# jerry102102102/RL_brain_trainer

Measured on AMD Instinct MI355X. Metric: env-steps/sec (whole node), Stage-5 Approach->Finisher PPO loops (rollout + update); value = the Approach loop, finisher.value = the Finisher loop, higher is better.
Workload: dtype f32

## Files before the change

### include/kp1_ppo.h

```cpp
#ifndef KP1_PPO_H
#define KP1_PPO_H

#include <stdint.h>

#include "kp1.h"

#ifdef __cplusplus
extern "C" {
#endif

int kp1_gae_scan(int32_t device, const float* rewards, const float* values, const uint8_t* dones, const float* last_values,
                 float gamma, float gae_lambda, float* advantages, float* returns, int32_t T, int32_t N, void* stream);

int kp1_gae_scan_replicas(int32_t device, const float* rewards, const float* values, const uint8_t* dones, const float* last_values,
                          const float* gamma_lambda, int32_t n_per_replica, float* advantages, float* returns, int32_t T, int32_t N, void* stream);

int kp1_bootstrap_truncated(int32_t device, float* rewards, const float* terminal_values, const uint8_t* dones, float gamma,
                            int64_t count, void* stream);

int kp1_adv_minibatch_sums(int32_t device, const float* advantages, const int64_t* idx, int64_t total, int64_t minibatch, double* out_sums,
                           void* stream);
int kp1_random_permutation(int32_t device, int64_t n, const uint32_t* keys, int64_t* out, void* stream);

int kp1_adv_minibatch_stats(int32_t device, const double* sums, int64_t n_minibatches, float* out_stats, void* stream);

#define KP1_CURRICULUM_MAX_WINDOW 1024
#define KP1_CURRICULUM_MAX_HISTORY 64
typedef struct kp1_curriculum_event {
  int64_t total_timesteps;
  int32_t from_stage, to_stage;
  double trigger_success_rate;
} kp1_curriculum_event;
typedef struct kp1_curriculum_state {
  int32_t stage_index;
  int32_t stage_episode_count;
  int32_t ring_len, ring_head;
  int32_t window_episodes, min_episodes_per_stage, max_stage_index, n_events;
  double success_rate_threshold;
  int64_t num_timesteps;
  int32_t ring[KP1_CURRICULUM_MAX_WINDOW];
  kp1_curriculum_event events[KP1_CURRICULUM_MAX_HISTORY];
} kp1_curriculum_state;

int kp1_curriculum_create(int32_t device, double success_rate_threshold, int32_t window_episodes, int32_t min_episodes_per_stage,
                          int32_t max_stage_index, int32_t initial_stage_index, kp1_curriculum_state** out_dev);
int kp1_curriculum_destroy(int32_t device, kp1_curriculum_state* st_dev);
int kp1_curriculum_observe(int32_t device, kp1_curriculum_state* st_dev, const uint8_t* dones, int32_t n, int32_t steps_per_call, void* stream);
int kp1_curriculum_observe_chunk(int32_t device, kp1_curriculum_state* st_dev, const uint8_t* dones, int32_t n_local, int32_t chunk_steps,
                                 int32_t world, void* stream);
int kp1_curriculum_read(int32_t device, const kp1_curriculum_state* st_dev, kp1_curriculum_state* out_host, void* stream);
int kp1_bind_stage_ptr(kp1_env* env, const int32_t* stage_dev);

#define KP1_CURRICULUM_MAX_REPLICAS 16
int kp1_curriculum_create_population(int32_t device, int32_t n_replicas, double success_rate_threshold, int32_t window_episodes,
                                     int32_t min_episodes_per_stage, int32_t max_stage_index, const int32_t* initial_stages,
                                     kp1_curriculum_state** out_dev);
int kp1_curriculum_observe_population(int32_t device, kp1_curriculum_state* states_dev, const uint8_t* dones, int32_t n_per_replica,
                                      int32_t n_replicas, int32_t steps_per_call, void* stream);
int kp1_curriculum_read_replica(int32_t device, const kp1_curriculum_state* states_dev, int32_t n_replicas, int32_t k,
                                kp1_curriculum_state* out_host, void* stream);
int kp1_bind_population_stages(kp1_env* env, const kp1_curriculum_state* states_dev, int32_t n_replicas);

#define KP1_DOCK_CURRICULUM_MAX_STAGES 16
#define KP1_DOCK_CURRICULUM_MAX_WINDOW 1024
#define KP1_DOCK_CURRICULUM_MAX_HISTORY 32
typedef struct kp1_dock_curriculum_stage {
  double action_delta_scale, dock_residual_action_limit, dock_delta_q_change_limit_scale;
  double close_bucket_probability, close_bucket_min_pos_error_m, close_bucket_max_pos_error_m, close_bucket_max_ori_error_rad,
         handoff_state_probability;
  double close_init_q_noise[KP1_NJ], init_q_noise[KP1_NJ];
  double success_rate_threshold;
  int32_t min_episodes;
  int32_t window_episodes;
  int32_t handoff_offset, handoff_count;
} kp1_dock_curriculum_stage;
typedef struct kp1_dock_curriculum_event {
  int64_t total_timesteps;
  int32_t from_stage, to_stage, stage_episode_count, reserved0;
  double trigger_success_rate;
} kp1_dock_curriculum_event;
typedef struct kp1_dock_curriculum_state {
  int32_t stage_index, stage_episode_count, ring_len, ring_head, window_episodes, n_stages, n_events, reserved0;
  int64_t num_timesteps;
  kp1_dock_curriculum_stage stages[KP1_DOCK_CURRICULUM_MAX_STAGES];
  kp1_dock_curriculum_event events[KP1_DOCK_CURRICULUM_MAX_HISTORY];
  uint8_t ring[KP1_DOCK_CURRICULUM_MAX_WINDOW];
} kp1_dock_curriculum_state;
int kp1_dock_curriculum_create(kp1_env* env, const kp1_dock_curriculum_stage* stages_host, int32_t n_stages, int32_t window_episodes,
                               kp1_dock_curriculum_state** out_dev);
int kp1_dock_curriculum_destroy(kp1_env* env, kp1_dock_curriculum_state* st_dev);
int kp1_dock_curriculum_observe(kp1_env* env, kp1_dock_curriculum_state* st_dev, const uint8_t* dones, int32_t n_local, int32_t chunk_steps, int32_t world,
                                void* stream);
int kp1_dock_curriculum_read(kp1_env* env, const kp1_dock_curriculum_state* st_dev, kp1_dock_curriculum_state* out_host, void* stream);
int kp1_dock_curriculum_create_population(kp1_env* env, const kp1_dock_curriculum_stage* stages_host, int32_t n_stages, int32_t window_episodes,
                                          int32_t n_replicas, kp1_dock_curriculum_state** out_dev);
int kp1_dock_curriculum_observe_population(kp1_env* env, kp1_dock_curriculum_state* states_dev, const uint8_t* dones, int32_t n_per_replica,
                                           int32_t n_replicas, void* stream);
int kp1_dock_curriculum_read_replica(kp1_env* env, const kp1_dock_curriculum_state* states_dev, int32_t n_replicas, int32_t k,
                                     kp1_dock_curriculum_state* out_host, void* stream);

#define KP1_MLP_IN 56
#define KP1_MLP_IN_PAD 64
#define KP1_MLP_IN_ROUTE 80
#define KP1_MLP_IN_ROUTE_PAD 128
#define KP1_MLP_ACT 7

typedef struct kp1_mlp kp1_mlp;

int kp1_mlp_create(int32_t device, int32_t hidden, int32_t max_batch, kp1_mlp** out);
int kp1_mlp_create_ex(int32_t device, int32_t hidden, int32_t obs_dim, int32_t max_batch, kp1_mlp** out);
#define KP1_MLP_MAX_REPLICAS 16
int kp1_mlp_create_population(int32_t device, int32_t hidden, int32_t obs_dim, int32_t max_batch, int32_t replicas, kp1_mlp** out);
int32_t kp1_mlp_replicas(const kp1_mlp* m);
typedef struct kp1_replica_hparams {
  float learning_rate, adam_eps, max_grad_norm, clip_range, ent_coef, vf_coef;
} kp1_replica_hparams;
int kp1_mlp_set_replica_hparams(kp1_mlp* m, const kp1_replica_hparams* host, int32_t n, void* stream);
int kp1_mlp_destroy(kp1_mlp* m);
int64_t kp1_mlp_num_params(int32_t hidden);
int64_t kp1_mlp_num_params_ex(int32_t hidden, int32_t obs_dim);
int kp1_mlp_pack_weights(kp1_mlp* m, const float* params, void* stream);

int kp1_mlp_forward(kp1_mlp* m, const float* obs, int32_t obs_stride, int32_t n, const float* noise, float* mean, float* value,
                    float* action, float* clipped_action, float* log_prob, void* stream);

int kp1_mlp_forward_env_step(kp1_mlp* m, kp1_env* env, const float* obs, int32_t obs_stride, const float* noise, float* value, float* action,
                             float* log_prob, float* next_obs, float* reward, uint8_t* done, float* terminal_obs, void* stream);

int kp1_mlp_loss_grad(kp1_mlp* m, const float* obs, int32_t obs_stride, const int64_t* idx, int32_t n, const float* actions,
                      const float* old_log_prob, const float* advantages, const float* returns, float adv_mean, float adv_inv_std,
                      const float* adv_stats_dev, float clip_range, float ent_coef, float vf_coef, float inv_count, float* grad_out,
                      float* stats_out, int32_t grad_is_zero, void* stream);

#define KP1_MLP_OPT_FUSED 1
#define KP1_MLP_OPT_ACTOR_EXTRA_STEPS 2
#define KP1_MLP_OPT_STEP_COUNT 3
#define KP1_MLP_OPT_PROFILE 4
#define KP1_MLP_OPT_BF16X3_WGRAD 5
#define KP1_MLP_PROFILE_SLOTS 4
#define KP1_MLP_PROFILE_TILE 0
#define KP1_MLP_PROFILE_WGRAD 1
#define KP1_MLP_PROFILE_FINALIZE 2
#define KP1_MLP_PROFILE_ADAM 3
int kp1_mlp_set_option(kp1_mlp* m, int32_t option, int32_t value);
int kp1_mlp_profile_read(kp1_mlp* m, float* out_us , int32_t* out_launches );

int kp1_mlp_adam_step(kp1_mlp* m, float* params, float* grad, float* exp_avg, float* exp_avg_sq, float lr, float eps,
                      float max_grad_norm, int32_t step, int32_t flags, void* stream);

int kp1_mlp_placement_check(int32_t device, int32_t n_rows, int32_t* out, void* stream);
int kp1_mlp_time_kernels(kp1_mlp* m, const float* obs, int32_t obs_stride, int32_t n, int32_t iters, float* out_ms, double* out_flops,
                         void* stream);

int kp1_set_obs_stride(kp1_env* env, int32_t stride);

#ifdef __cplusplus
}
#endif
#endif
```

### rl_brain_trainer_amd/csrc/kp1_env_step.inc

```

#ifdef KP1_ENV_TRACE
constexpr int KP1_ENV_TRACE_SLOTS = 16, KP1_ENV_TRACE_WAVES = 1024;
__device__ unsigned long long kp1_env_trace_buf[KP1_ENV_TRACE_SLOTS * KP1_ENV_TRACE_WAVES];
__device__ __forceinline__ void etr_pin(float v) { asm volatile("" ::"v"(v)); }
__device__ __forceinline__ void etr_pin(double v) { asm volatile("" ::"v"(v)); }
__device__ __forceinline__ void etr_pin(int v) { asm volatile("" ::"v"(v)); }
#define KP1_ETR_PIN(slot, ...)                                                                                                    \
  {                                                                                                                               \
    for (auto pv_ : {__VA_ARGS__}) etr_pin(pv_);                                                                                  \
    __builtin_amdgcn_sched_barrier(0);                                                                                            \
    KP1_ETR(slot)                                                                                                                 \
    __builtin_amdgcn_sched_barrier(0);                                                                                            \
  }
#define KP1_ETR(slot)                                                                                                             \
  {                                                                                                                               \
    const unsigned long long t_ = __builtin_readcyclecounter();                                                                   \
    const int w_ = (int)((blockIdx.x * blockDim.x + threadIdx.x) >> 6);                                                           \
    if ((threadIdx.x & 63) == 0 && w_ < KP1_ENV_TRACE_WAVES) kp1_env_trace_buf[w_ * KP1_ENV_TRACE_SLOTS + (slot)] = t_;           \
  }
#else
#define KP1_ETR(slot)
#define KP1_ETR_PIN(slot, ...)
#endif

// ... 198 lines not shown
    for (int k = 0; k < 6; ++k) goal_pose[k] = (R)opts.goal_pose6[i * 6 + k];
#pragma unroll
    for (int k = 0; k < NJ; ++k) goal_q[k] = (opts.flags & OPT_GOAL_Q) ? (R)opts.goal_q[i * NJ + k] : (R)0;
  } else if (opts.flags & OPT_GOAL_Q) {
#pragma unroll
    for (int k = 0; k < NJ; ++k) {
      gq64[k] = dclip(opts.goal_q[i * NJ + k], smp.lower[k], smp.upper[k]);
      goal_q[k] = (R)gq64[k];
    }
    fk_pose6_kin<R>(cfg.kin.fk, gq64, goal_pose);
  } else if (!given_q) {
#pragma unroll
    for (int k = 0; k < NJ; ++k) goal_q[k] = (R)rs.goal_q[k];
    if (sampled_goal_pose) {
#pragma unroll
      for (int k = 0; k < 6; ++k) goal_pose[k] = (R)rs.goal_pose6[k];
    } else {
      fk_pose6_kin<R>(cfg.kin.fk, rs.goal_q, goal_pose);
    }
  } else {
    rng_load(st.rng64, st.rng32, n, i, rng);
    rng_used = true;
    double g[NJ];
    sample_joint_configuration(smp, rng, smp.goal_sample_margin_fraction, g);
#pragma unroll
    for (int k = 0; k < NJ; ++k) goal_q[k] = (R)g[k];
    fk_pose6_kin<R>(cfg.kin.fk, g, goal_pose);
  }
  if (rng_used) rng_store(st.rng64, st.rng32, n, i, rng);
  R pe[3], oe[3], pn, on;
  pose_error_norms<R>(ee, goal_pose, pe, oe, &pn, &on);
#pragma unroll
  for (int k = 0; k < NJ; ++k) {
    st.q_store(k, i, q64[k]);
    st.r(F_DQ + k, i) = dq[k];
    st.r(F_PREV_ACTION + k, i) = pa[k];
    st.r(F_GOAL_Q + k, i) = goal_q[k];
  }
#pragma unroll
  for (int k = 0; k < 6; ++k) {
    st.r(F_GOAL_POSE + k, i) = goal_pose[k];
    st.r(F_EE_POSE + k, i) = ee[k];
  }
  st.r(F_ENTRY + 0, i) = pn;
  st.r(F_ENTRY + 1, i) = on;
  st.r(F_ENTRY + 2, i) = norm7<R>(pa);
  st.r(F_ENTRY + 3, i) = norm7<R>(dq);
  st.r(F_MIN_POS, i) = std::numeric_limits<R>::infinity();
  st.r(F_POS_ERR, i) = pn;
  st.r(F_ORI_ERR, i) = on;
  st.r(F_EXEC_DQ, i) = (R)0;
  st.r(F_ACTION_L2, i) = (R)0;
  st.r(F_DQ_CHANGE, i) = (R)0;
  st.iv(I_STEP, i) = 0;
  st.iv(I_DWELL, i) = 0;
  st.iv(I_ENTRY, i) = 0;
  st.iv(I_DRIFT, i) = 0;
  st.iv(I_FLAGS, i) = 0;
  st.iv(I_STAGE, i) = have_sample ? rs.stage : stage_index;
  build_observation<R>(cfg, MODE, q, dq, pa, pe, oe, 0, 0, o);
}

template <typename R>
struct StepArgs {
  EnvState<R> st;
  const DevCfg<R>* cfg;
  const DevSampler* smp;
  const kp1_handoff_state* handoff;
  const R* actions;
  float* obs;
  R* reward;
  uint8_t* done;
  float* terminal_obs;
  R* comps;
  int auto_reset;
  int stage_index;
  int obs_stride;
  const int32_t* stage_ptr;
  const kp1_curriculum_state* pop_states;
  int n_per_replica;
  const kp1_dock_curriculum_stage* pop_dock;
};

template <typename R, int MODE, bool COMPS, bool POP = false>
__device__ __forceinline__ void step_env_lane(const StepArgs<R>& a, const int64_t i, const R* __restrict__ act_src, float* __restrict__ o) {
  const int64_t n = a.st.n;
  KP1_ETR(0)
  const DevCfg<R>& __restrict__ cfg = *scalar_cache_warm(a.cfg);
  const DevFk<double>& __restrict__ fkc = cfg.kin.fk;
  KP1_ETR(1)
  const EnvState<R>& st = a.st;
  const R Z = (R)0;

  R act[NJ], dq[NJ], prev_action[NJ], goal[6], ee[6];
  double q[NJ];
#pragma unroll
  for (int k = 0; k < NJ; ++k) {
    act[k] = kp_clip<R>(act_src[k], (R)-1, (R)1);
    q[k] = st.q_loadl(k, i);
    dq[k] = st.rl(F_DQ + k, i);
    prev_action[k] = st.rl(F_PREV_ACTION + k, i);
  }
#pragma unroll
  for (int k = 0; k < 6; ++k) {
    goal[k] = st.rl(F_GOAL_POSE + k, i);
    ee[k] = st.rl(F_EE_POSE + k, i);
  }
  int episode_step = st.ivl(I_STEP, i), dwell = st.ivl(I_DWELL, i), entry_count = st.ivl(I_ENTRY, i), drift_count = st.ivl(I_DRIFT, i);
  int flags = st.ivl(I_FLAGS, i);
  R min_pos = st.rl(F_MIN_POS, i);

  R pe[3], oe[3], prev_pos, prev_ori;
  pose_error_norms<R>(ee, goal, pe, oe, &prev_pos, &prev_ori);
  KP1_ETR_PIN(2, prev_pos, prev_ori)

  constexpr bool LIVE = POP && MODE == KP1_MODE_DOCK;
  const kp1_dock_curriculum_stage* __restrict__ live = nullptr;
  if constexpr (LIVE) live = a.pop_dock + (uint32_t)i / (uint32_t)a.n_per_replica;
  R dyn_limit = kp_clip<R>(cfg.env.dock_residual_action_limit, Z, (R)1);
  R dyn_dqc = kp_max<R>(cfg.env.dock_delta_q_change_limit_scale, Z);
  if constexpr (MODE == KP1_MODE_DOCK) {
    const R residual_limit = LIVE ? (R)live->dock_residual_action_limit : cfg.env.dock_residual_action_limit;
    const R dqc_limit_scale = LIVE ? (R)live->dock_delta_q_change_limit_scale : cfg.env.dock_delta_q_change_limit_scale;
    dyn_limit = kp_clip<R>(interpolate_control<R>(prev_pos, cfg.env.dock_dynamic_action_limit_near_pos_threshold_m,
                                                  cfg.env.dock_dynamic_action_limit_far_pos_threshold_m,
                                                  cfg.env.dock_dynamic_residual_action_limit_near,
                                                  cfg.env.dock_dynamic_residual_action_limit_far, residual_limit), Z, (R)1);
    dyn_dqc = kp_max<R>(interpolate_control<R>(prev_pos, cfg.env.dock_dynamic_action_limit_near_pos_threshold_m,
                                               cfg.env.dock_dynamic_action_limit_far_pos_threshold_m,
                                               cfg.env.dock_dynamic_delta_q_change_limit_scale_near,
                                               cfg.env.dock_dynamic_delta_q_change_limit_scale_far, dqc_limit_scale), Z);
#pragma unroll
    for (int k = 0; k < NJ; ++k) act[k] = kp_clip<R>(act[k], -dyn_limit, dyn_limit);
  }
  const bool prev_in_near = is_near_goal<R>(cfg, prev_pos, prev_ori);
  double scale = LIVE ? live->action_delta_scale : cfg.kin.action_delta_scale;
  if constexpr (MODE == KP1_MODE_DOCK) {
    if (cfg.kin.dock_action_delta_scale > 0.0) scale = cfg.kin.dock_action_delta_scale;
  } else {
    if (cfg.env.dynamic_action_delta_scale_enabled) {
      R mult = interpolate_control<R>(prev_pos, cfg.env.dynamic_action_delta_scale_near_pos_threshold_m,
                                      cfg.env.dynamic_action_delta_scale_far_pos_threshold_m,
                                      cfg.env.dynamic_action_delta_scale_near_multiplier,
                                      cfg.env.dynamic_action_delta_scale_far_multiplier, (R)1);
      scale = cfg.kin.action_delta_scale * (double)kp_max<R>(mult, Z);
    }
  }
  R q_next[NJ], dq_next[NJ];
  double q_next64[NJ];
  R dq_change_ss = Z, dq_ss = Z, prev_dq_ss = Z, act_ss = Z, pact_ss = Z, dact_ss = Z, margin_min = (R)1;
#pragma unroll
  for (int k = 0; k < NJ; ++k) {
    const double max_dq = cfg.kin.dlim[k] * scale;
    double cmd = (double)act[k] * max_dq;
    if constexpr (MODE == KP1_MODE_DOCK) {
      if (dyn_dqc > Z) {
        const double lim = max_dq * (double)dyn_dqc, dqk = (double)dq[k];
        cmd = dqk + dclip(cmd - dqk, -lim, lim);
        cmd = dclip(cmd, -max_dq, max_dq);
      }
    }
    q_next64[k] = joint_clip<double>(q[k] + cmd, cfg.kin.lower[k], cfg.kin.upper[k]);
    q_next[k] = (R)q_next64[k];
    dq_next[k] = (R)(q_next64[k] - q[k]);
    R dd = dq_next[k] - dq[k];
    dq_change_ss += dd * dd;
    dq_ss += dq_next[k] * dq_next[k];
    prev_dq_ss += dq[k] * dq[k];
    act_ss += act[k] * act[k];
    pact_ss += prev_action[k] * prev_action[k];
    R da = act[k] - prev_action[k];
    dact_ss += da * da;
    margin_min = kp_min<R>(margin_min, joint_limit_margin<R>(q_next[k], cfg.lower[k], cfg.upper[k]));
  }
  KP1_ETR_PIN(3, q_next64[0], q_next64[1], q_next64[2], q_next64[3], q_next64[4], q_next64[5], q_next64[6], (double)margin_min, (double)dq_change_ss)
  R ee_next[6];
  fk_pose6_kin<R>(fkc, q_next64, ee_next);
  KP1_ETR_PIN(4, ee_next[0], ee_next[1], ee_next[2], ee_next[3], ee_next[4], ee_next[5])
  R curr_pos, curr_ori;
  pose_error_norms<R>(ee_next, goal, pe, oe, &curr_pos, &curr_ori);
  const bool curr_pre = is_pre_near_goal<R>(cfg, curr_pos, curr_ori);
  const bool curr_near = is_near_goal<R>(cfg, curr_pos, curr_ori);
  min_pos = curr_pos < min_pos ? curr_pos : min_pos;
  if (curr_pre) flags |= FLAG_PRE_NEAR_HIT;
  if (curr_near && !prev_in_near) entry_count += 1;
  dwell = curr_near ? dwell + 1 : 0;
  if (prev_in_near && curr_pos > prev_pos) drift_count += 1;

  const int step_count = episode_step + 1;
  bool terminated = false, truncated = false, success = false, invalid = false;
  const bool criteria = curr_pos <= cfg.term.success_pos_threshold_m &&
                        (!cfg.term.require_orientation || curr_ori <= cfg.term.success_ori_threshold_rad) &&
                        dwell >= cfg.term.success_dwell_steps;
  if (!kp_isfinite(curr_pos) || !kp_isfinite(curr_ori)) {
    terminated = true;
    invalid = true;
  } else if (criteria) {
    success = true;
    if (cfg.term.terminate_on_success) terminated = true;
  }
  if (!terminated && step_count >= cfg.term.max_episode_steps) truncated = true;

  KP1_ETR_PIN(5, curr_pos, curr_ori, (R)dwell, (R)(terminated ? 1 : 0), (R)(truncated ? 1 : 0))
  RewardIn<R> ri;
  ri.prev_pos = prev_pos; ri.curr_pos = curr_pos; ri.prev_ori = prev_ori; ri.curr_ori = curr_ori;
  ri.action_norm = kp_sqrt(act_ss); ri.prev_action_norm = kp_sqrt(pact_ss);
  ri.action_msq = kp_div(act_ss, (R)7); ri.action_delta_msq = kp_div(dact_ss, (R)7);
  ri.dq_norm = kp_sqrt(dq_ss); ri.prev_dq_norm = kp_sqrt(prev_dq_ss); ri.dq_change_l2 = kp_sqrt(dq_change_ss);
  ri.margin_min = margin_min;
  ri.dwell = dwell; ri.entry_count = entry_count; ri.drift_count = drift_count;
  ri.pre = curr_pre; ri.cn = curr_near; ri.pn = prev_in_near; ri.success = success;
  R reward;
  if constexpr (MODE == KP1_MODE_DOCK) {
    ri.entry_pos = st.r(F_ENTRY + 0, i); ri.entry_ori = st.r(F_ENTRY + 1, i);
    ri.entry_action = st.r(F_ENTRY + 2, i); ri.entry_dq = st.r(F_ENTRY + 3, i);
    reward = dock_reward<R, COMPS>(cfg.dock, ri, COMPS ? a.comps + i : nullptr, n);
  } else {
    ri.entry_pos = ri.entry_ori = ri.entry_action = ri.entry_dq = Z;
    reward = approach_reward<R, COMPS>(cfg.reward, ri, COMPS ? a.comps + i : nullptr, n);
  }
  KP1_ETR_PIN(6, reward)
  episode_step += 1;
  if (curr_near) flags |= FLAG_NEAR_HIT;
  flags = success ? (flags | FLAG_SUCCESS) : (flags & ~FLAG_SUCCESS);

  build_observation<R>(cfg, MODE, q_next, dq_next, act, pe, oe, episode_step, dwell, o);
  KP1_ETR_PIN(7, o[0], o[7], o[14], o[21], o[28], o[31], o[34], o[40], o[54], o[55], o[6], o[13], o[20], o[27])
  a.reward[i] = reward;
  const bool done = terminated || truncated;
  a.done[i] = (uint8_t)((terminated ? KP1_DONE_TERMINATED : 0) | (truncated ? KP1_DONE_TRUNCATED : 0) |
                        (success ? KP1_DONE_SUCCESS : 0) | (invalid ? KP1_DONE_INVALID : 0));
  if (done && a.auto_reset) {
    if (a.terminal_obs) store_obs_row(a.terminal_obs, i, o, a.obs_stride);
    ResetOptsDev none = {nullptr, nullptr, nullptr, nullptr, nullptr, 0};
    int stage = a.stage_index;
    const DevSampler& smp = uniform_block(a.smp);
    if constexpr (POP && !LIVE) stage = kp_clipi(a.pop_states[(uint32_t)i / (uint32_t)a.n_per_replica].stage_index, 0, kp_maxi(smp.n_stages - 1, 0));
    else if (a.stage_ptr) stage = kp_clipi(*a.stage_ptr, 0, kp_maxi(smp.n_stages - 1, 0));
    reset_env<R, MODE, LIVE>(st, cfg, smp, a.handoff, none, stage, i, o, live);
    st.r(F_POS_ERR, i) = curr_pos;
    st.r(F_ORI_ERR, i) = curr_ori;
    st.r(F_EXEC_DQ, i) = ri.dq_norm;
    st.r(F_ACTION_L2, i) = ri.action_norm;
    st.r(F_DQ_CHANGE, i) = ri.dq_change_l2;
    st.iv(I_FLAGS, i) = (flags & FLAG_SUCCESS);
  } else {
#pragma unroll
    for (int k = 0; k < NJ; ++k) {
      st.q_store(k, i, q_next64[k]);
      st.r(F_DQ + k, i) = dq_next[k];
      st.r(F_PREV_ACTION + k, i) = act[k];
    }
#pragma unroll
    for (int k = 0; k < 6; ++k) st.r(F_EE_POSE + k, i) = ee_next[k];
    st.r(F_MIN_POS, i) = min_pos;
    st.r(F_POS_ERR, i) = curr_pos;
    st.r(F_ORI_ERR, i) = curr_ori;
    st.r(F_EXEC_DQ, i) = ri.dq_norm;
    st.r(F_ACTION_L2, i) = ri.action_norm;
    st.r(F_DQ_CHANGE, i) = ri.dq_change_l2;
    st.iv(I_STEP, i) = episode_step;
    st.iv(I_DWELL, i) = dwell;
    st.iv(I_ENTRY, i) = entry_count;
    st.iv(I_DRIFT, i) = drift_count;
    st.iv(I_FLAGS, i) = flags;
  }
  KP1_ETR(10)
}
```

### rl_brain_trainer_amd/csrc/kp1_mlp.hip

```cpp
#include <hip/hip_runtime.h>
#include <hip/hip_ext.h>

#include <cmath>
#include <cstddef>
#include <cstdlib>
#include <cstring>
#include <vector>

#include "../../include/kp1_ppo.h"
#include "kp1_device.hpp"
#include "kp1_host.hpp"

using kp1::fail;
using namespace kp1;

typedef float f32x16 __attribute__((ext_vector_type(16)));
typedef float f32x4 __attribute__((ext_vector_type(4)));

namespace {

constexpr int ACT = KP1_MLP_ACT, HEADS = 8;
constexpr float LOG_SQRT_2PI = 0.9189385332046727f;

enum { EPI_BIAS_TANH = 0, EPI_DTANH = 1 };
// ... 974 lines not shown
  __syncthreads();
  for (int k = 128; k > 0; k >>= 1) {
    if (threadIdx.x < k) s[threadIdx.x] += s[threadIdx.x + k];
    __syncthreads();
  }
  if (threadIdx.x == 0) partials[blockIdx.x] = s[0];
}

constexpr int ADAM_BLOCK = 256, VEC = 1;
template <bool POP = false>
__global__ void __launch_bounds__(ADAM_BLOCK) adam_kernel(float* __restrict__ p, float* __restrict__ g, float* __restrict__ m, float* __restrict__ v,
                                                   int64_t n, const double* __restrict__ partials, int n_partials, float lr, float eps, float max_norm,
                                                   float bc1, float bc2_sqrt, const ParamLayout L, const Packed k_, int zero_grad,
                                                   const int* __restrict__ step_counter, int host_step, const int* __restrict__ actor_extra,
                                                   unsigned r_partials, const float* __restrict__ hparams) {
  __shared__ float scale_s;
  const Packed k = POP ? packed_replica(k_, L, blockIdx.y) : k_;
  if constexpr (POP) {
    const unsigned o = blockIdx.y * (unsigned)n;
    p += o; g += o; m += o; v += o;
    partials += blockIdx.y * r_partials;
    if (hparams) {
      const float* e = hparams + blockIdx.y * (unsigned)HP_FIELDS;
      lr = e[HP_LR];
      eps = e[HP_EPS];
      max_norm = e[HP_MAX_NORM];
    }
  }
  const int64_t i0 = ((int64_t)blockIdx.x * ADAM_BLOCK + threadIdx.x) * VEC;
  float g_in[VEC], m_in[VEC], v_in[VEC], p_in[VEC];
#pragma unroll
  for (int j = 0; j < VEC; ++j) {
    const int64_t il = i0 + j < n ? i0 + j : n - 1;
    g_in[j] = g[il]; m_in[j] = m[il]; v_in[j] = v[il]; p_in[j] = p[il];
  }
  const int extra = *actor_extra;
  float base_step = (float)host_step;
  if (step_counter) base_step = (float)*step_counter;
  double s = 0.0;
  if (threadIdx.x < 64) {
    for (int q = threadIdx.x; q < n_partials; q += 64) s += partials[q];
    for (int off = 32; off > 0; off >>= 1) s += __shfl_xor(s, off);
  }
  if (threadIdx.x == 0) {
    const float norm = (float)sqrt(s);
    scale_s = max_norm > 0.f ? fminf(max_norm / (norm + 1e-6f), 1.f) : 1.f;
  }
  if (step_counter) {
    bc1 = 1.f - powf(0.9f, base_step);
    bc2_sqrt = sqrtf(1.f - powf(0.999f, base_step));
  }
  float bc1_a = bc1, bc2_sqrt_a = bc2_sqrt;
  if (extra != 0) {
    const float st = base_step + (float)extra;
    bc1_a = 1.f - powf(0.9f, st);
    bc2_sqrt_a = sqrtf(1.f - powf(0.999f, st));
  }
  __syncthreads();
  const float scale = scale_s;
  float pn[VEC], mn[VEC], vn[VEC];
#pragma unroll
  for (int j = 0; j < VEC; ++j) {
    const int64_t i = i0 + j;
    const bool actor = extra != 0 && ((i >= L.p_w1 && i < L.v_w1) || (i >= L.a_w && i < L.c_w));
    const float b1 = actor ? bc1_a : bc1, b2 = actor ? bc2_sqrt_a : bc2_sqrt;
    const float gi = g_in[j] * scale;
    mn[j] = 0.9f * m_in[j] + 0.1f * gi;
    vn[j] = 0.999f * v_in[j] + 0.001f * gi * gi;
    const float denom = sqrtf(vn[j]) / b2 + eps;
    pn[j] = p_in[j] - (lr / b1) * (mn[j] / denom);
  }
#pragma unroll
  for (int j = 0; j < VEC; ++j) {
    const int64_t i = i0 + j;
    if (i < n) {
      m[i] = mn[j]; v[i] = vn[j]; p[i] = pn[j];
      pack_one(i, pn[j], L, k);
      if (zero_grad) g[i] = 0.f;
    }
  }
}

#include "kp1_env_step.inc"
#include "kp1_mlp_tile.inc"
#include "kp1_mlp_fused.inc"

}

struct kp1_mlp {
  int device = 0, H = 0, Hp = 0, max_batch = 0;
  int K = 1;
  ParamLayout L;
  Packed k{};
  float* h1 = nullptr;
  float* h2 = nullptr;
  float* dz2 = nullptr;
  float* dz1 = nullptr;
  float* xf = nullptr;
  int bf16x3 = 0;
  unsigned short* sp_h1 = nullptr; unsigned short* sp_dz2 = nullptr; unsigned short* sp_dz1 = nullptr; unsigned short* sp_xf = nullptr;
  double* partials = nullptr;
  float* slab = nullptr;
  float* slab1 = nullptr;
  float* bslab = nullptr;
  float* hpart = nullptr;
  int n_finalize_blocks = 0;
  int* step_dev = nullptr;
  float* hparams_dev = nullptr;
  bool hparams_on = false;
  int last_s2_n = 0, last_s1_n = 0;
  int fused = 1;
  const float* last_params = nullptr;
  bool slab_stale = false;
  std::vector<void*> allocs;
  int profile = 0;
  struct ProfPair { hipEvent_t a, b; };
  std::vector<ProfPair> prof[KP1_MLP_PROFILE_SLOTS];
  int prof_used[KP1_MLP_PROFILE_SLOTS] = {0, 0, 0, 0};
};

namespace {
struct ProfSlotInFlight { hipEvent_t a = nullptr, b = nullptr; bool attached = false; };
thread_local ProfSlotInFlight tl_prof;

struct ProfScope {
  kp1_mlp* m; int slot; hipStream_t stream; bool on;
  ProfScope(kp1_mlp* m_, int slot_, hipStream_t s_) : m(m_), slot(slot_), stream(s_), on(m_->profile != 0) {
    if (!on) return;
    auto& v = m->prof[slot];
    if (m->prof_used[slot] >= (int)v.size()) {
      kp1_mlp::ProfPair p{};
      if (hipEventCreate(&p.a) != hipSuccess || hipEventCreate(&p.b) != hipSuccess) { on = false; return; }
      v.push_back(p);
    }
    tl_prof.a = v[m->prof_used[slot]].a;
    tl_prof.b = v[m->prof_used[slot]].b;
    tl_prof.attached = false;
  }
  ~ProfScope() {
    if (!on) return;
    if (!tl_prof.attached) {
      (void)hipEventRecord(tl_prof.a, stream);
      (void)hipEventRecord(tl_prof.b, stream);
    }
    tl_prof = ProfSlotInFlight{};
    m->prof_used[slot] += 1;
  }
};

#define KP1_LAUNCH(kernel, grid, block, bytes, stream, ...)                                                        \
  do {                                                                                                             \
    if (tl_prof.a != nullptr && !tl_prof.attached) {                                                               \
      tl_prof.attached = true;                                                                                     \
      hipExtLaunchKernelGGL(kernel, grid, block, bytes, stream, tl_prof.a, tl_prof.b, 0, __VA_ARGS__);             \
    } else {                                                                                                       \
      hipLaunchKernelGGL(kernel, grid, block, bytes, stream, __VA_ARGS__);                                         \
    }                                                                                                              \
  } while (0)
}

namespace {

constexpr int N_PARTIALS = 128;
constexpr int PARTIALS_STRIDE = 2 * N_PARTIALS + 2048;
constexpr int TN_SPLIT2 = 8, TN_SPLIT1 = 16;

// ... 340 lines not shown
    HIP_TRY(hipMemcpy(m->step_dev + 1, &value, sizeof(int), hipMemcpyHostToDevice));
    return KP1_OK;
  }
  return fail(KP1_ERR_INVALID, "unknown kp1_mlp option");
}

int kp1_mlp_set_replica_hparams(kp1_mlp* m, const kp1_replica_hparams* host, int32_t n, void* stream) {
  static_assert(sizeof(kp1_replica_hparams) == sizeof(float) * HP_FIELDS, "kp1_replica_hparams is HP_FIELDS floats");
  static_assert(offsetof(kp1_replica_hparams, learning_rate) == sizeof(float) * HP_LR && offsetof(kp1_replica_hparams, adam_eps) == sizeof(float) * HP_EPS &&
                offsetof(kp1_replica_hparams, max_grad_norm) == sizeof(float) * HP_MAX_NORM && offsetof(kp1_replica_hparams, clip_range) == sizeof(float) * HP_CLIP &&
                offsetof(kp1_replica_hparams, ent_coef) == sizeof(float) * HP_ENT && offsetof(kp1_replica_hparams, vf_coef) == sizeof(float) * HP_VF,
                "kp1_replica_hparams field order");
  if (!m) return fail(KP1_ERR_INVALID, "NULL argument");
  if (n == 0) {
    m->hparams_on = false;
    return KP1_OK;
  }
  if (m->K == 1) return fail(KP1_ERR_UNSUPPORTED, "a K = 1 handle takes its hyper-parameters as scalar arguments, not a per-replica table");
  if (n != m->K || !host) return fail(KP1_ERR_INVALID, "kp1_mlp_set_replica_hparams needs one entry per replica (n = K)");
  for (int r = 0; r < n; ++r) {
    const kp1_replica_hparams& h = host[r];
    for (float v : {h.learning_rate, h.adam_eps, h.max_grad_norm, h.clip_range, h.ent_coef, h.vf_coef})
      if (!std::isfinite(v)) return fail(KP1_ERR_INVALID, "replica hyper-parameters must be finite");
  }
  int rc = mlp_check_device(m);
  if (rc != KP1_OK) return rc;
  HIP_TRY(hipMemcpyAsync(m->hparams_dev, host, sizeof(kp1_replica_hparams) * (size_t)n, hipMemcpyHostToDevice, (hipStream_t)stream));
  HIP_TRY(hipStreamSynchronize((hipStream_t)stream));
  m->hparams_on = true;
  return KP1_OK;
}

int kp1_mlp_pack_weights(kp1_mlp* m, const float* params, void* stream) {
  if (!m || !params) return fail(KP1_ERR_INVALID, "NULL argument");
  int rc = mlp_check_device(m);
  if (rc != KP1_OK) return rc;
  Packed k = m->k;
  k.formats = PACK_SLAB | PACK_FRAG;
  if (m->K > 1)
    hipLaunchKernelGGL(pack_kernel<true>, dim3((unsigned)((m->L.total + 255) / 256), m->K), dim3(256), 0, (hipStream_t)stream, params, m->L, k);
  else
    hipLaunchKernelGGL(pack_kernel<false>, dim3((unsigned)((m->L.total + 255) / 256)), dim3(256), 0, (hipStream_t)stream, params, m->L, k);
  HIP_TRY(kp1::launch_status());
  m->last_params = params;
  m->slab_stale = false;
  return KP1_OK;
}

int kp1_mlp_forward(kp1_mlp* m, const float* obs, int32_t obs_stride, int32_t n, const float* noise, float* mean, float* value, float* action,
                    float* clipped_action, float* log_prob, void* stream) {
  if (!m || !obs) return fail(KP1_ERR_INVALID, "NULL argument");
  if (n <= 0 || n > m->max_batch) return fail(KP1_ERR_INVALID, "n exceeds the workspace max_batch");
  const int IN = m->L.IN, INP = m->L.INP;
  if (obs_stride != IN && obs_stride != INP) return fail(KP1_ERR_INVALID, "obs_stride must be the observation width or its padded width (56 / 64, or 80 / 128)");
  int rc = mlp_check_device(m);
  if (rc != KP1_OK) return rc;
  if (m->fused && m->Hp == FU_HP) {
    FusedArgs fa{};
    fa.obs = obs; fa.obs_stride = obs_stride; fa.Kreal = obs_stride >= INP ? INP : IN; fa.inp = INP; fa.idx = nullptr; fa.n = n;
    fa.k = m->k;
    fa.noise = noise; fa.mean = mean; fa.value = value; fa.action = action; fa.clipped = clipped_action; fa.log_prob = log_prob;
    rc = launch_fused_infer(fa, (hipStream_t)stream);
    if (rc != KP1_OK) return rc;
    HIP_TRY(kp1::launch_status());
    return KP1_OK;
  }
  rc = launch_forward_layers(m, obs, obs_stride, nullptr, n, (hipStream_t)stream);
  if (rc != KP1_OK) return rc;
  HeadArgs a{};
  a.h2 = m->h2; a.strideH = (int64_t)m->max_batch * m->Hp; a.Hp = m->Hp; a.n = n; a.H = m->H;
  a.w3 = m->k.w3; a.b3 = m->k.b3; a.log_std = m->k.log_std;
  a.noise = noise; a.mean = mean; a.value = value; a.action = action; a.clipped = clipped_action; a.log_prob = log_prob;
  if (m->K > 1) {
    a.r_act = (unsigned)(2 * a.strideH);
    hipLaunchKernelGGL(head_infer_kernel<true>, dim3((n + HEAD_ROWS - 1) / HEAD_ROWS, m->K), dim3(256), sizeof(float) * HEADS * m->Hp, (hipStream_t)stream, a);
  } else {
    hipLaunchKernelGGL(head_infer_kernel<false>, dim3((n + HEAD_ROWS - 1) / HEAD_ROWS), dim3(256), sizeof(float) * HEADS * m->Hp, (hipStream_t)stream, a);
  }
  HIP_TRY(kp1::launch_status());
  return KP1_OK;
}

int kp1_mlp_forward_env_step(kp1_mlp* m, kp1_env* env, const float* obs, int32_t obs_stride, const float* noise, float* value, float* action,
                             float* log_prob, float* next_obs, float* reward, uint8_t* done, float* terminal_obs, void* stream) {
  if (!m || !env || !obs || !action || !next_obs || !reward || !done) return fail(KP1_ERR_INVALID, "NULL argument to kp1_mlp_forward_env_step");
  if (m->K > 1) return fail(KP1_ERR_UNSUPPORTED, "kp1_mlp_forward_env_step is not available on population handles");
  if (!(m->fused && m->Hp == FU_HP) || m->L.INP != 64)
    return fail(KP1_ERR_UNSUPPORTED, "kp1_mlp_forward_env_step needs the 2x256 tile kernels and the 56-float observation (padded to 64)");
  if (obs_stride != m->L.IN && obs_stride != m->L.INP) return fail(KP1_ERR_INVALID, "obs_stride must be 56 or 64");
  int rc = mlp_check_device(m);
  if (rc != KP1_OK) return rc;
  FusedArgs fa{};
  int mode = 0, device = 0;
  int64_t n_envs = 0;
  rc = kp1::env_step_args_f32(env, &fa.env, sizeof fa.env, nullptr, next_obs, reward, done, terminal_obs, 1, &mode, &n_envs, &device);
  if (rc != KP1_OK) return rc;
  if (device != m->device) return fail(KP1_ERR_INVALID, "the env handle and the MLP workspace live on different devices");
  if (n_envs > m->max_batch) return fail(KP1_ERR_INVALID, "more envs than the workspace max_batch");
  fa.obs = obs; fa.obs_stride = obs_stride; fa.Kreal = obs_stride >= m->L.INP ? m->L.INP : m->L.IN; fa.inp = m->L.INP; fa.idx = nullptr; fa.n = (int)n_envs;
  fa.k = m->k;
  fa.noise = noise; fa.value = value; fa.action = action; fa.log_prob = log_prob;
  rc = launch_fused_infer_env(fa, mode, (hipStream_t)stream);
  if (rc != KP1_OK) return rc;
  HIP_TRY(kp1::launch_status());
  return KP1_OK;
}

int kp1_mlp_loss_grad(kp1_mlp* m, const float* obs, int32_t obs_stride, const int64_t* idx, int32_t n, const float* actions,
                      const float* old_log_prob, const float* advantages, const float* returns, float adv_mean, float adv_inv_std,
                      const float* adv_stats_dev, float clip_range, float ent_coef, float vf_coef, float inv_count, float* grad_out,
                      float* stats_out, int32_t grad_is_zero, void* stream_) {
  if (!m || !obs || !actions || !old_log_prob || !advantages || !returns || !grad_out) return fail(KP1_ERR_INVALID, "NULL argument");
  if (n <= 0 || n > m->max_batch) return fail(KP1_ERR_INVALID, "n exceeds the workspace max_batch");
  const int IN = m->L.IN, INP = m->L.INP;
  if (obs_stride != IN && obs_stride != INP) return fail(KP1_ERR_INVALID, "obs_stride must be the observation width or its padded width (56 / 64, or 80 / 128)");
  int rc = mlp_check_device(m);
  if (rc != KP1_OK) return rc;
  hipStream_t stream = (hipStream_t)stream_;
  const int Hp = m->Hp, H = m->H;
  const int64_t act_stride = (int64_t)m->max_batch * Hp;
  const ParamLayout& L = m->L;
  (void)grad_is_zero;
  const bool fused = m->fused && Hp == FU_HP;
  const bool pop = m->K > 1;
  if (pop && !idx) return fail(KP1_ERR_INVALID, "population handles gather their rows through idx [K][n]");
  const int64_t hpart_rep = (int64_t)(m->max_batch / 32) * (10 * Hp + 32);
  int adv_mode = 0;
  if (adv_stats_dev) adv_mode = 2;
  else if (adv_inv_std > 0.f) adv_mode = 3;
  else if (adv_inv_std == 0.f) adv_mode = 1;
  if (adv_mode == 1) {
    if (pop)
      hipLaunchKernelGGL(adv_partials_kernel<true>, dim3(N_PARTIALS, m->K), dim3(256), 0, stream, advantages, idx, n, m->partials, (unsigned)PARTIALS_STRIDE);
    else
      hipLaunchKernelGGL(adv_partials_kernel<false>, dim3(N_PARTIALS), dim3(256), 0, stream, advantages, idx, n, m->partials, 0u);
  }
  const int hpart_stride = 10 * Hp + 32;
  if (fused) {
    FusedArgs fa{};
    fa.obs = obs; fa.obs_stride = obs_stride; fa.Kreal = obs_stride >= INP ? INP : IN; fa.inp = INP; fa.idx = idx; fa.n = n;
    fa.k = m->k;
    fa.actions = actions; fa.old_logp = old_log_prob; fa.adv = advantages; fa.ret = returns;
    fa.adv_partials = m->partials; fa.n_adv_partials = N_PARTIALS; fa.adv_stats = adv_stats_dev; fa.adv_mean = adv_mean; fa.adv_inv_std = adv_inv_std;
    fa.adv_mode = adv_mode;
    fa.clip_range = clip_range; fa.vf_coef = vf_coef; fa.inv_count = inv_count;
    fa.h1 = m->h1; fa.dz2 = m->dz2; fa.dz1 = m->dz1; fa.act_stride = act_stride; fa.xf = m->xf;
    fa.bslab = m->bslab; fa.hpart = m->hpart; fa.hpart_stride = hpart_stride;
    if (m->bf16x3) {
      fa.sp_h1 = m->sp_h1; fa.sp_dz2 = m->sp_dz2; fa.sp_dz1 = m->sp_dz1; fa.sp_xf = m->sp_xf;
      fa.sp_plane = (int64_t)2 * m->max_batch * Hp; fa.sp_plane_x = (int64_t)m->max_batch * INP;
    }
    {
      ProfScope ps(m, KP1_MLP_PROFILE_TILE, stream);
      rc = launch_fused(fa, stream);
    }
    if (rc != KP1_OK) return rc;
  } else {
    rc = launch_forward_layers(m, obs, obs_stride, idx, n, stream);
    if (rc != KP1_OK) return rc;
    HeadArgs a{};
    a.h2 = m->h2; a.strideH = act_stride; a.Hp = Hp; a.n = n; a.H = H;
    a.w3 = m->k.w3; a.b3 = m->k.b3; a.log_std = m->k.log_std;
    a.idx = idx; a.actions = actions; a.old_logp = old_log_prob; a.adv = advantages; a.ret = returns;
    a.adv_partials = m->partials; a.n_adv_partials = N_PARTIALS; a.adv_stats = adv_stats_dev; a.adv_mean = adv_mean; a.adv_inv_std = adv_inv_std;
    a.adv_mode = adv_mode;
    a.clip_range = clip_range; a.ent_coef = ent_coef; a.vf_coef = vf_coef; a.inv_count = inv_count;
    a.dz2 = m->dz2;
    a.hpart = m->hpart; a.hpart_stride = hpart_stride;
    a.r_act = (unsigned)(2 * act_stride); a.r_hpart = (unsigned)hpart_rep; a.r_partials = (unsigned)PARTIALS_STRIDE;
    a.hparams = pop && m->hparams_on ? m->hparams_dev : nullptr;
    {
      const dim3 hgrid((n + HEAD_ROWS - 1) / HEAD_ROWS, m->K);
      const size_t hbytes = sizeof(float) * (HEADS * Hp + HEAD_ROWS * 8 + 84 + 2 * HEAD_ROWS * (Hp + 4));
      if (pop) {
        HIP_TRY(hipFuncSetAttribute((const void*)head_train_kernel<128, true>, hipFuncAttributeMaxDynamicSharedMemorySize, (int)hbytes));
        hipLaunchKernelGGL((head_train_kernel<128, true>), hgrid, dim3(256), hbytes, stream, a);
      } else if (Hp == 256) {
        HIP_TRY(hipFuncSetAttribute((const void*)head_train_kernel<256>, hipFuncAttributeMaxDynamicSharedMemorySize, (int)hbytes));
        hipLaunchKernelGGL(head_train_kernel<256>, hgrid, dim3(256), hbytes, stream, a);
      } else {
        HIP_TRY(hipFuncSetAttribute((const void*)head_train_kernel<128>, hipFuncAttributeMaxDynamicSharedMemorySize, (int)hbytes));
        hipLaunchKernelGGL(head_train_kernel<128>, hgrid, dim3(256), hbytes, stream, a);
      }
    }
// ... 321 lines not shown
```

### rl_brain_trainer_amd/csrc/kp1_mlp_tile.inc

```

struct FusedArgs {
  const float* obs; int64_t obs_stride; int Kreal;
  int inp;
  const int64_t* idx; int n;
  Packed k;
  const float* actions; const float* old_logp; const float* adv; const float* ret;
  const double* adv_partials; int n_adv_partials; const float* adv_stats; float adv_mean, adv_inv_std; int adv_mode;
  float clip_range, vf_coef, inv_count;
  float* h1; float* dz2; float* dz1; int64_t act_stride;
  float* xf;
  float* bslab;
  float* hpart; int hpart_stride;
  const float* noise; float* mean; float* value; float* action; float* clipped; float* log_prob;
  int net_base;
  int stagger_ticks, n_cus;
  StepArgs<float> env;
  unsigned short* sp_h1; unsigned short* sp_dz2; unsigned short* sp_dz1; unsigned short* sp_xf; int64_t sp_plane, sp_plane_x;
};

typedef __bf16 bf16x8 __attribute__((ext_vector_type(8)));
struct Split3 { bf16x8 hi, mid, lo; };
__device__ __forceinline__ Split3 split3(const float* v) {
  Split3 o;
#pragma unroll
  for (int j = 0; j < 8; ++j) {
    const __bf16 h = (__bf16)v[j];
    const float r1 = v[j] - (float)h;
    const __bf16 m = (__bf16)r1;
    const float r2 = r1 - (float)m;
    o.hi[j] = h;
    o.mid[j] = m;
    o.lo[j] = (__bf16)r2;
  }
  return o;
}
__device__ __forceinline__ void store_split3(unsigned short* __restrict__ base, int64_t plane, int64_t fi, int ncb, int cb, int lane, const Split3& s) {
  const int64_t at = ((fi * ncb + cb) * 64 + lane) * 8;
  *reinterpret_cast<bf16x8*>(base + at) = s.hi;
  *reinterpret_cast<bf16x8*>(base + plane + at) = s.mid;
  *reinterpret_cast<bf16x8*>(base + 2 * plane + at) = s.lo;
}

__host__ __device__ inline int64_t frag8_at(int64_t b, int64_t col, int64_t C) {
  return ((b >> 3) * (C >> 5) + (col >> 5)) * 256 + ((col & 31) + 32 * ((b & 7) >> 2)) * 4 + (b & 3);
}

__device__ __forceinline__ f32x4 fu_wload(const char* __restrict__ base, unsigned off) {
  const __amdgpu_buffer_rsrc_t r = __builtin_amdgcn_make_buffer_rsrc(const_cast<char*>(base), 0, 0x7fffffff, 0x00020000);
  return __builtin_bit_cast(f32x4, __builtin_amdgcn_raw_buffer_load_b128(r, (int)off, 0, AUX_SC1));
}
constexpr int FU_HP = 256, FU_BKS = 32, FU_AP = FU_HP + 4;
constexpr int FU_STAGE = FU_HP * FU_BKS;
constexpr int FU_BM = 32, FU_NW = 4, FU_CB = 2, FU_NTH = 64 * FU_NW;
constexpr int FU_SCRATCH = 4 * FU_BM * 8 + FU_BM * 8 + FU_NW * 24 + 64;
constexpr int FU_LDS_FLOATS = 2 * FU_BM * FU_AP + HEADS * FU_HP + FU_SCRATCH;
static_assert(FU_LDS_FLOATS * 4 * 2 <= 160 * 1024, "the two training tiles of one CU must fit its LDS");

template <bool TRAIN, int K1S, int ENV = 0, bool SPLIT = false>
__global__ void __launch_bounds__(FU_NTH, ENV ? 1 : 2) mlp_tile_kernel(const FusedArgs a) {
  static_assert(!(TRAIN && ENV), "the env step rides on the inference tile only");
  static_assert(TRAIN || !SPLIT, "split planes are written by the training tile");
  constexpr int NW = FU_NW, CB = FU_CB, BM = FU_BM, NTH = FU_NTH, CW = 32 * CB;
  constexpr int INP = K1S * FU_BKS, FU_XP = INP + 4, GS_L2 = K1S, GS_BW = K1S + 8, GS_END = K1S + 16;
  constexpr int KG = FU_BKS / 8, NB = CB * KG;
  constexpr int L1_REAL_GROUPS = K1S == 2 ? (KP1_MLP_IN + 7) / 8 : (KP1_MLP_IN_ROUTE + 7) / 8;
  extern __shared__ float lds[];
  float* bufA = lds;
  float* bufB = bufA + BM * FU_AP;
  float* w3s = bufB + BM * FU_AP;
  float* dotred = w3s + HEADS * FU_HP;
  float* dout = dotred + 4 * BM * 8;
  float* wsum = dout + BM * 8;
  float* misc = wsum + NW * 24;

  const int z = (int)blockIdx.z + a.net_base;
  const int m0 = blockIdx.x * BM, slot = blockIdx.x;
  const int tid = threadIdx.x, lane = tid & 63, wave = __builtin_amdgcn_readfirstlane(tid >> 6);
  const unsigned lane_off = (unsigned)lane * 16u;
  const char* __restrict__ W1F = reinterpret_cast<const char*>(a.k.w1f + (int64_t)z * K1S * FU_STAGE + wave * NB * 64 * 4);
  const char* __restrict__ W2F = reinterpret_cast<const char*>(a.k.w2f + (int64_t)z * 8 * FU_STAGE + wave * NB * 64 * 4);
  const char* __restrict__ W2TF = reinterpret_cast<const char*>(a.k.w2tf + (int64_t)z * 8 * FU_STAGE + wave * NB * 64 * 4);

  f32x4 bf[3][NB];
#define FU_BLOAD(gs)                                                                                    \
  if ((gs) < GS_END) {                                                                                  \
    const char* p_ = (gs) < GS_L2 ? W1F + (gs) * (FU_STAGE * 4) : ((gs) < GS_BW ? W2F + ((gs) - GS_L2) * (FU_STAGE * 4) : W2TF + ((gs) - GS_BW) * (FU_STAGE * 4)); \
    _Pragma("unroll") for (int q = 0; q < NB; ++q) bf[(gs) % 3][q] = fu_wload(p_, q * 1024 + lane_off); \
  }
  f32x16 acc[CB];
#define FU_INIT_ACC(bias)                                                                               \
  _Pragma("unroll") for (int c = 0; c < CB; ++c)                                                        \
    _Pragma("unroll") for (int e = 0; e < 16; ++e) acc[c][e] = (bias)[c];
#ifdef KP1_TR_HEADS
#define KP1_TR_G2(slot)
#define KP1_TR_HD(slot) KP1_TR(slot)
#else
#define KP1_TR_G2(slot) KP1_TR(slot)
#define KP1_TR_HD(slot)
#endif
#ifdef KP1_FU_NOMFMA
#define FU_MFMA(acc_, a_, b_) acc_[0] += (a_) * (b_);
#else
#define FU_MFMA(acc_, a_, b_) acc_ = __builtin_amdgcn_mfma_f32_32x32x2f32(a_, b_, acc_, 0, 0, 0);
#endif
#ifdef KP1_FU_NOTANH
#define FU_TANH(x) (x)
#else
#define FU_TANH(x) kp_tanh(x)
#endif
#define FU_GEMM(abuf, ap, KT, GS0)                                                                      \
  {                                                                                                     \
    const float* as = (abuf) + (lane & 31) * (ap) + 4 * (lane >> 5);                                     \
    _Pragma("unroll") for (int s = 0; s < (KT); ++s) {                                                  \
      FU_BLOAD((GS0) + s + 2)                                                                           \
      __builtin_amdgcn_sched_barrier(0);                                                                \
      f32x4 av[KG];                                                                                     \
      _Pragma("unroll") for (int kg = 0; kg < KG; ++kg)                                                 \
        av[kg] = *reinterpret_cast<const f32x4*>(as + s * FU_BKS + kg * 8);                              \
      _Pragma("unroll") for (int kg = 0; kg < KG; ++kg)                                                 \
        if (!((GS0) == 0 && s * KG + kg >= L1_REAL_GROUPS))    \
        _Pragma("unroll") for (int i = 0; i < 4; ++i)                                                   \
          _Pragma("unroll") for (int c = 0; c < CB; ++c)                                                \
            FU_MFMA(acc[c], av[kg][i], bf[((GS0) + s) % 3][c * KG + kg][i])                              \
      __builtin_amdgcn_sched_barrier(0);                                                                \
      if ((GS0) == GS_L2) { KP1_TR_G2(7 + s) }                                                          \
    }                                                                                                   \
  }
#define FU_ROW(e) (((e) & 3) + 8 * ((e) >> 2) + 4 * (lane >> 5))
#define FU_COL(c) (wave * CW + (c) * 32 + (lane & 31))
#ifdef KP1_FU_NOSTORE
#define FU_STORE_ACC(dst)
#else
#define FU_STORE_ACC(dst)                                                                               \
  _Pragma("unroll") for (int c = 0; c < CB; ++c)                                                        \
    _Pragma("unroll") for (int g = 0; g < 4; ++g) {                                                     \
      const f32x4 v_ = {acc[c][4 * g], acc[c][4 * g + 1], acc[c][4 * g + 2], acc[c][4 * g + 3]};        \
      *reinterpret_cast<f32x4*>((dst) + ((int64_t)((m0 >> 3) + g) * (FU_HP / 32) + wave * CB + c) * 256 + lane * 4) = v_; \
    }
#endif
// ... 16 lines not shown
      store_split3((dst) + (zoff), (plane), (int64_t)(m0 >> 4) + f_, (C) / 32, cb_, lane, split3(v8_));  \
    }                                                                                                   \
  }
#ifdef KP1_FU_NOSTORE
#define FU_STORE_FRAG(tile, pitch, dst, C)
#else
#define FU_STORE_FRAG(tile, pitch, dst, C)                                                              \
  _Pragma("unroll") for (int q = wave; q < (BM / 8) * ((C) / 32); q += NW) {                            \
    const int g_ = q / ((C) / 32), cb_ = q % ((C) / 32);                                                \
    const float* t_ = (tile) + (8 * g_ + 4 * (lane >> 5)) * (pitch) + 32 * cb_ + (lane & 31);           \
    f32x4 v_;                                                                                           \
    _Pragma("unroll") for (int i = 0; i < 4; ++i) v_[i] = t_[i * (pitch)];                              \
    *reinterpret_cast<f32x4*>((dst) + ((int64_t)((m0 >> 3) + g_) * ((C) / 32) + cb_) * 256 + lane * 4) = v_; \
  }
#endif

  KP1_TR(0)
  if (TRAIN) { KP1_CLK(0, 0) }
  if (TRAIN && a.stagger_ticks > 0) {
    const int linear = blockIdx.x + gridDim.x * blockIdx.z;
    if (linear >= a.n_cus && linear < 2 * a.n_cus) {
      const unsigned long long t0_ = wall_clock64();
      while (wall_clock64() - t0_ < (unsigned long long)a.stagger_ticks) __builtin_amdgcn_s_sleep(16);
    }
  }
  FU_BLOAD(0)
  FU_BLOAD(1)
  __builtin_amdgcn_sched_barrier(0);
  {
    constexpr int XQ = INP / 4, X_LOADS = BM * XQ / NTH;
    constexpr int W3_LOADS = HEADS * FU_HP / 4 / NTH;
    static_assert(X_LOADS >= 1 && X_LOADS * NTH == BM * XQ && W3_LOADS >= 1 && W3_LOADS * NTH == HEADS * FU_HP / 4, "prologue loads must tile the workgroup");
    int64_t xrow[X_LOADS];
    f32x4 xv[X_LOADS], w3v[W3_LOADS];
#pragma unroll
    for (int j = 0; j < X_LOADS; ++j) {
      const int m = min(m0 + (tid + NTH * j) / XQ, a.n - 1);
      xrow[j] = a.idx ? a.idx[m] : (int64_t)m;
    }
#pragma unroll
    for (int j = 0; j < X_LOADS; ++j) {
      const int k = 4 * ((tid + NTH * j) % XQ);
      xv[j] = *reinterpret_cast<const f32x4*>(a.obs + xrow[j] * a.obs_stride + (k < a.Kreal ? k : 0));
    }
#pragma unroll
    for (int j = 0; j < W3_LOADS; ++j) w3v[j] = *reinterpret_cast<const f32x4*>(a.k.w3 + 4 * (tid + NTH * j));
#pragma unroll
    for (int j = 0; j < X_LOADS; ++j) {
      const int f = tid + NTH * j, row = f / XQ, k = 4 * (f % XQ);
      const float keep = (m0 + row < a.n && k < a.Kreal) ? 1.f : 0.f;
      *reinterpret_cast<f32x4*>(bufB + row * FU_XP + k) = xv[j] * keep;
    }
#pragma unroll
    for (int j = 0; j < W3_LOADS; ++j) *reinterpret_cast<f32x4*>(w3s + 4 * (tid + NTH * j)) = w3v[j];
  }
  if (TRAIN && z == 0 && wave == 0) {
    float mean = 0.f, inv_std = 1.f;
    if (a.adv_mode == 1) {
      double ps = 0.0, pss = 0.0;
      for (int k = lane; k < a.n_adv_partials; k += 64) {
        ps += a.adv_partials[2 * k];
        pss += a.adv_partials[2 * k + 1];
      }
      for (int off = 32; off > 0; off >>= 1) {
        ps += __shfl_xor(ps, off);
        pss += __shfl_xor(pss, off);
      }
      const double mu = ps / a.n;
      const double var = a.n > 1 ? fmax((pss - a.n * mu * mu) / (a.n - 1), 0.0) : 0.0;
      mean = (float)mu;
      inv_std = (float)(1.0 / (sqrt(var) + 1e-8));
    } else if (a.adv_mode == 2) {
      mean = a.adv_stats[0];
      inv_std = a.adv_stats[1];
    } else if (a.adv_mode == 3) {
      mean = a.adv_mean;
      inv_std = a.adv_inv_std;
    }
    if (lane == 0) {
      misc[0] = mean;
      misc[1] = inv_std;
    }
  }
  float bias1[CB], bias2[CB];
#pragma unroll
  for (int c = 0; c < CB; ++c) {
    bias1[c] = a.k.b1[z * FU_HP + FU_COL(c)];
    bias2[c] = a.k.b2[z * FU_HP + FU_COL(c)];
  }
  const int l_row = tid >> 3, l_out = tid & 7;
  const bool l_ok = m0 + l_row < a.n;
  const int64_t l_src = a.idx ? a.idx[min(m0 + l_row, a.n - 1)] : (int64_t)min(m0 + l_row, a.n - 1);
  __syncthreads();
  KP1_TR(1)
  constexpr bool fp32_out = !SPLIT;
  if (TRAIN && z == 0 && fp32_out) { FU_STORE_FRAG(bufB, FU_XP, a.xf, INP) }
  if (TRAIN && z == 0) { FU_STORE_FRAG_SPLIT(bufB, FU_XP, a.sp_xf, a.sp_plane_x, (int64_t)0, INP) }

  FU_INIT_ACC(bias1)
  FU_GEMM(bufB, FU_XP, K1S, 0)
#pragma unroll
  for (int c = 0; c < CB; ++c)
#pragma unroll
    for (int e = 0; e < 16; ++e) {
      acc[c][e] = FU_TANH(acc[c][e]);
      bufA[FU_ROW(e) * FU_AP + FU_COL(c)] = acc[c][e];
    }
  if (TRAIN && fp32_out) { FU_STORE_ACC(a.h1 + z * a.act_stride) }
  if (TRAIN) { FU_STORE_ACC_SPLIT(a.sp_h1, a.sp_plane) }
  __syncthreads();
  KP1_TR(2)
  float l_act = 0.f, l_old = 0.f, l_adv = 0.f, l_ret = 0.f, l_b3 = a.k.b3[l_out], l_ls = a.k.log_std[l_out < ACT ? l_out : 0];
  if (TRAIN) {
    if (z == 0) {
      if (l_out < ACT) l_act = a.actions[l_src * ACT + l_out];
      l_old = a.old_logp[l_src];
      l_adv = a.adv[l_src];
    } else {
      l_ret = a.ret[l_src];
    }
  } else if (z == 0 && a.noise && l_ok && l_out < ACT) {
    l_act = a.noise[l_src * ACT + l_out];
  }

  FU_INIT_ACC(bias2)
  FU_GEMM(bufA, FU_AP, 8, GS_L2)
#pragma unroll
  for (int c = 0; c < CB; ++c)
#pragma unroll
    for (int e = 0; e < 16; ++e) bufB[FU_ROW(e) * FU_AP + FU_COL(c)] = FU_TANH(acc[c][e]);
  __syncthreads();
  KP1_TR(3)

  {
    const int row = lane & 31, kq = wave, part = kq * 2 + (lane >> 5);
    const float* hrow = bufB + row * FU_AP + part * 32;
    f32x4 hv[8];
#pragma unroll
    for (int q = 0; q < 8; ++q) hv[q] = *reinterpret_cast<const f32x4*>(hrow + 4 * q);
    auto dot = [&](int o) {
      const float* w = w3s + o * FU_HP + part * 32;
      float s = 0.f;
#pragma unroll
      for (int q = 0; q < 8; ++q) {
        const f32x4 wv = *reinterpret_cast<const f32x4*>(w + 4 * q);
        s = fmaf(hv[q].x, wv.x, s);
        s = fmaf(hv[q].y, wv.y, s);
        s = fmaf(hv[q].z, wv.z, s);
        s = fmaf(hv[q].w, wv.w, s);
      }
      s += __shfl_xor(s, 32);
      if (lane < 32) dotred[(kq * BM + row) * 8 + o] = s;
    };
    if (z == 0) {
#pragma unroll
      for (int o = 0; o < ACT; ++o) dot(o);
    } else {
      dot(7);
    }
  }
  __syncthreads();
  KP1_TR_HD(7)
  if (!TRAIN) {
    const bool mine = z == 0 ? l_out < ACT : l_out == 7;
    float v = 0.f;
    if (mine) {
#pragma unroll
      for (int p = 0; p < 4; ++p) v += dotred[(p * BM + l_row) * 8 + l_out];
      v += l_b3;
    }
    float lp = 0.f;
    if (z == 0) {
      float act = v;
      if (l_ok && l_out < ACT) {
        if (a.mean) a.mean[l_src * ACT + l_out] = v;
        if (a.noise) {
          act = fmaf(expf(l_ls), l_act, v);
          lp = -0.5f * l_act * l_act - l_ls - LOG_SQRT_2PI;
        }
        if (a.action) a.action[l_src * ACT + l_out] = act;
        if (a.clipped) a.clipped[l_src * ACT + l_out] = fminf(fmaxf(act, -1.f), 1.f);
      }
      lp += __shfl_xor(lp, 1);
      lp += __shfl_xor(lp, 2);
      lp += __shfl_xor(lp, 4);
      if (l_ok && l_out == 0 && a.log_prob) a.log_prob[l_src] = lp;
      if constexpr (ENV != 0) {
        dout[l_row * 8 + l_out] = (l_ok && l_out < ACT) ? act : 0.f;
        __syncthreads();
        if (wave == 0) {
          const bool live = lane < BM && m0 + lane < a.n;
          float o[KP1_OBS_DIM];
          if (live) step_env_lane<float, ENV == 1 ? KP1_MODE_APPROACH : KP1_MODE_DOCK, false>(a.env, (int64_t)(m0 + lane), dout + lane * 8, o);
          store_obs_tile(a.env.obs, (int64_t)m0, min(BM, a.n - m0), o, live, a.env.obs_stride, bufA);
        }
      }
    } else if (l_ok && l_out == 7 && a.value) {
      a.value[l_src] = v;
    }
    return;
  }
  {
    const int row_l = l_row, out = l_out;
    const bool ok = l_ok;
    const bool mine = z == 0 ? out < ACT : out == 7;
    float v = 0.f;
    if (mine) {
#pragma unroll
      for (int p = 0; p < 4; ++p) v += dotred[(p * BM + row_l) * 8 + out];
      v += l_b3;
    }
    float zs = 0.f, inv_sd = 1.f, lp = 0.f;
    if (z == 0 && ok && out < ACT) {
      inv_sd = expf(-l_ls);
      zs = (l_act - v) * inv_sd;
      lp = -0.5f * zs * zs - l_ls - LOG_SQRT_2PI;
    }
    lp += __shfl_xor(lp, 1);
    lp += __shfl_xor(lp, 2);
    lp += __shfl_xor(lp, 4);
    float g_logp = 0.f, d = 0.f, pl = 0.f, vl = 0.f, kl = 0.f;
    if (ok && z == 0) {
      const float A = (l_adv - misc[0]) * misc[1];
      const float lr_ = lp - l_old;
      const float ratio = expf(lr_);
      const float rc = fminf(fmaxf(ratio, 1.f - a.clip_range), 1.f + a.clip_range);
      const float s1 = ratio * A, s2 = rc * A;
      const bool inside = ratio >= 1.f - a.clip_range && ratio <= 1.f + a.clip_range;
      g_logp = (inside || s1 < s2) ? -A * ratio * a.inv_count : 0.f;
      if (out < ACT) {
        d = g_logp * zs * inv_sd;
      } else {
        pl = -fminf(s1, s2);
        kl = (ratio - 1.f) - lr_;
      }
    } else if (ok && out == 7) {
      d = a.vf_coef * 2.f * (v - l_ret) * a.inv_count;
      vl = (l_ret - v) * (l_ret - v);
    }
    dout[row_l * 8 + out] = (ok && mine) ? d : 0.f;
    float gls = (z == 0 && ok && out < ACT) ? g_logp * (zs * zs - 1.f) : 0.f;
    float dsum = (ok && mine) ? d : 0.f;
    float l0 = pl, l1 = vl, l2 = kl;
#pragma unroll
    for (int off = 8; off < 64; off <<= 1) {
      gls += __shfl_xor(gls, off);
      dsum += __shfl_xor(dsum, off);
      l0 += __shfl_xor(l0, off);
      l1 += __shfl_xor(l1, off);
      l2 += __shfl_xor(l2, off);
    }
    if (lane < 8) {
      wsum[wave * 24 + out] = dsum;
      wsum[wave * 24 + 8 + out] = gls;
      if (out == 7) {
        wsum[wave * 24 + 16] = l0;
        wsum[wave * 24 + 17] = l1;
        wsum[wave * 24 + 18] = l2;
      }
    }
  }
  KP1_TR_HD(8)
  __syncthreads();
  KP1_TR_HD(9)
  if (tid < 18) {
    const int k = tid;
    const int w = k < 8 ? k : (k < 15 ? 8 + (k - 8) : 16 + (k - 15));
    const float v = ((wsum[w] + wsum[24 + w]) + wsum[48 + w]) + wsum[72 + w];
    const bool pi_slot = (k < 7) || (k >= 8 && k < 15) || k == 15 || k == 17;
    if (pi_slot == (z == 0)) a.hpart[(int64_t)slot * a.hpart_stride + 10 * FU_HP + k] = v;
  }
  {
    constexpr int DZ_COLS = FU_HP / NW, DZ_CG = DZ_COLS / 4, DZ_RG = 64 / DZ_CG, DZ_ROWS = 32 / DZ_RG;
    const int cg = lane % DZ_CG, rg = lane / DZ_CG, col = wave * DZ_COLS + 4 * cg;
    float* part = a.hpart + (int64_t)slot * a.hpart_stride;
    f32x4 gw[ACT], gb2 = {0.f, 0.f, 0.f, 0.f}, w3c[ACT];
#pragma unroll
// ... 102 lines not shown
```

### rl_brain_trainer_amd/csrc/kp1_ppo.hip

```cpp
#include <hip/hip_runtime.h>

#include <cstring>
#include <vector>

#include "../../include/kp1_ppo.h"
#include "kp1_host.hpp"

using kp1::fail;

namespace {

__global__ void __launch_bounds__(256) gae_scan_kernel(const float* __restrict__ rewards, const float* __restrict__ values,
                                                       const uint8_t* __restrict__ dones, const float* __restrict__ last_values,
                                                       float gamma, float lam, float* __restrict__ adv, float* __restrict__ ret, int T, int N) {
  const int i = blockIdx.x * blockDim.x + threadIdx.x;
  if (i >= N) return;
  float next_value = last_values[i];
  float last_gae = 0.0f;
  for (int t = T - 1; t >= 0; --t) {
    const int64_t k = (int64_t)t * N + i;
    const float nonterm = (dones[k] & (KP1_DONE_TERMINATED | KP1_DONE_TRUNCATED)) ? 0.0f : 1.0f;
    const float v = values[k];
    const float delta = rewards[k] + gamma * next_value * nonterm - v;
    last_gae = delta + gamma * lam * nonterm * last_gae;
    adv[k] = last_gae;
    ret[k] = last_gae + v;
    next_value = v;
  }
}

__global__ void __launch_bounds__(256) gae_scan_replicas_kernel(const float* __restrict__ rewards, const float* __restrict__ values,
                                                                const uint8_t* __restrict__ dones, const float* __restrict__ last_values,
                                                                const float* __restrict__ gamma_lambda, int n_per_replica, float* __restrict__ adv,
                                                                float* __restrict__ ret, int T, int N) {
  const int i = blockIdx.x * blockDim.x + threadIdx.x;
  if (i >= N) return;
  const int r = i / n_per_replica;
  const float gamma = gamma_lambda[2 * r], lam = gamma_lambda[2 * r + 1];
  float next_value = last_values[i];
  float last_gae = 0.0f;
  for (int t = T - 1; t >= 0; --t) {
    const int64_t k = (int64_t)t * N + i;
    const float nonterm = (dones[k] & (KP1_DONE_TERMINATED | KP1_DONE_TRUNCATED)) ? 0.0f : 1.0f;
    const float v = values[k];
    const float delta = rewards[k] + gamma * next_value * nonterm - v;
    last_gae = delta + gamma * lam * nonterm * last_gae;
    adv[k] = last_gae;
    ret[k] = last_gae + v;
    next_value = v;
  }
}

__global__ void __launch_bounds__(256) bootstrap_kernel(float* __restrict__ rewards, const float* __restrict__ tv,
                                                        const uint8_t* __restrict__ dones, float gamma, int64_t count) {
  const int64_t k = (int64_t)blockIdx.x * blockDim.x + threadIdx.x;
  if (k >= count) return;
  const uint8_t d = dones[k];
  if ((d & KP1_DONE_TRUNCATED) && !(d & KP1_DONE_TERMINATED)) rewards[k] += gamma * tv[k];
}

struct TrackerCtx {
  int stage, count, len, head, window, min_episodes, max_stage, n_events, sum;
  double threshold;
  long long timesteps;
  bool ring_dirty;
};

__device__ __forceinline__ void tracker_load(const kp1_curriculum_state* __restrict__ st, int* __restrict__ ring, TrackerCtx& c) {
  const int lane = threadIdx.x;
  c.stage = st->stage_index; c.count = st->stage_episode_count; c.len = st->ring_len; c.head = st->ring_head;
  c.window = st->window_episodes; c.min_episodes = st->min_episodes_per_stage; c.max_stage = st->max_stage_index; c.n_events = st->n_events;
  c.threshold = st->success_rate_threshold; c.timesteps = st->num_timesteps;
  c.ring_dirty = false;
  int part = 0;
  for (int k = lane; k < c.window; k += 64) {
    const int v = st->ring[k];
    ring[k] = v;
    const int age = k >= c.head ? k - c.head : k - c.head + c.window;
    if (age < c.len) part += v;
  }
  for (int off = 32; off > 0; off >>= 1) part += __shfl_xor(part, off);
  c.sum = part;
  __syncthreads();
}

__device__ __forceinline__ void tracker_store(kp1_curriculum_state* __restrict__ st, const int* __restrict__ ring, const TrackerCtx& c) {
  const int lane = threadIdx.x;
  __syncthreads();
  if (c.ring_dirty)
    for (int k = lane; k < c.window; k += 64) st->ring[k] = ring[k];
  if (lane == 0) {
    st->stage_index = c.stage; st->stage_episode_count = c.count; st->ring_len = c.len; st->ring_head = c.head;
    st->n_events = c.n_events; st->num_timesteps = c.timesteps;
  }
}

constexpr int TRK_BLOCK = 64 * 64, TRK_PARALLEL_MIN = 192;
struct TrackerScratch { uint8_t* sbit; uint16_t* pfx; };

__device__ __forceinline__ void tracker_append_run(int* __restrict__ ring, TrackerCtx& c, const uint8_t* __restrict__ sbit, int pos, int R) {
  const int lane = threadIdx.x, W = c.window;
  const int j0 = R > W ? R - W : 0;
  __syncthreads();
  for (int j = j0 + lane; j < R; j += 64) ring[(c.head + c.len + j) % W] = sbit[pos + j];
  __syncthreads();
  const int over = c.len + R - W;
  c.head = over > 0 ? (c.head + over) % W : c.head;
  c.len = c.len + R < W ? c.len + R : W;
  c.count += R;
  int part = 0;
  for (int k = lane; k < W; k += 64) {
    const int age = k >= c.head ? k - c.head : k - c.head + W;
    if (age < c.len) part += ring[k];
  }
  for (int off = 32; off > 0; off >>= 1) part += __shfl_xor(part, off);
  c.sum = part;
}

__device__ __forceinline__ void tracker_block_parallel(kp1_curriculum_state* __restrict__ st, int* __restrict__ ring, TrackerCtx& c, const TrackerScratch& ws,
                                                       unsigned long long dmask, unsigned long long smask, int E) {
  const int lane = threadIdx.x, W = c.window;
  int mine = __popcll(dmask), off = mine;
  for (int d = 1; d < 64; d <<= 1) {
    const int up = __shfl_up(off, d);
    if (lane >= d) off += up;
  }
  off -= mine;
  __syncthreads();
  for (unsigned long long m = dmask; m; m &= m - 1) {
    const int b = __ffsll((long long)m) - 1;
    ws.sbit[off++] = (uint8_t)((smask >> b) & 1ull);
  }
  __syncthreads();
  int pos = 0;
  while (pos < E) {
    const int R = E - pos;
    if (c.stage >= c.max_stage) {
      tracker_append_run(ring, c, ws.sbit, pos, R);
      break;
    }
    const int L = c.len, T = L + R;
    const int seg = (T + 63) / 64, j_lo = lane * seg < T ? lane * seg : T, j_hi = j_lo + seg < T ? j_lo + seg : T;
    auto y = [&](int j) -> int { return j < L ? ring[(c.head + j) % W] : (int)ws.sbit[pos + (j - L)]; };
    int tot = 0;
    for (int j = j_lo; j < j_hi; ++j) tot += y(j);
    int run = tot;
    for (int d = 1; d < 64; d <<= 1) {
      const int up = __shfl_up(run, d);
      if (lane >= d) run += up;
    }
    run -= tot;
    __syncthreads();
    if (lane == 0) ws.pfx[0] = 0;
    for (int j = j_lo; j < j_hi; ++j) {
      run += y(j);
      ws.pfx[j + 1] = (uint16_t)run;
    }
    __syncthreads();
    int best = R;
    for (int r = lane; r < R; r += 64) {
      const int filled = L + r + 1;
      if (filled < W || c.count + r + 1 < c.min_episodes) continue;
      const int wsum = (int)ws.pfx[filled] - (int)ws.pfx[filled - W];
      if ((double)wsum / (double)W >= c.threshold) {
        best = r;
        break;
      }
    }
    for (int d = 32; d > 0; d >>= 1) {
      const int o = __shfl_xor(best, d);
      best = o < best ? o : best;
    }
    if (best >= R) {
      tracker_append_run(ring, c, ws.sbit, pos, R);
      break;
    }
    const int filled = L + best + 1;
    const double rate = (double)((int)ws.pfx[filled] - (int)ws.pfx[filled - W]) / (double)W;
    if (lane == 0 && c.n_events < KP1_CURRICULUM_MAX_HISTORY) {
      kp1_curriculum_event& ev = st->events[c.n_events];
      ev.total_timesteps = c.timesteps;
      ev.from_stage = c.stage;
      ev.to_stage = c.stage + 1;
      ev.trigger_success_rate = rate;
    }
    c.n_events += 1;
    c.stage += 1;
    c.count = 0;
    c.len = 0;
    c.head = 0;
    c.sum = 0;
    pos += best + 1;
  }
}

__device__ __forceinline__ void curriculum_scan(kp1_curriculum_state* __restrict__ st, int* __restrict__ ring, TrackerCtx& c, const TrackerScratch& ws,
                                                const uint8_t* __restrict__ dones, int n, int steps_per_call) {
  const int lane = threadIdx.x;
  c.timesteps += steps_per_call;
  for (int base = 0; base < n; base += 64 * 64) {
    const int first = base + lane * 64;
    unsigned long long dmask = 0ull, smask = 0ull;
    if (first + 64 <= n && (reinterpret_cast<uintptr_t>(dones + first) & 15) == 0) {
      const uint4* p = reinterpret_cast<const uint4*>(dones + first);
      uint4 w[4];
#pragma unroll
      for (int q = 0; q < 4; ++q) w[q] = p[q];
#pragma unroll
      for (int q = 0; q < 4; ++q) {
        const unsigned int words[4] = {w[q].x, w[q].y, w[q].z, w[q].w};
#pragma unroll
        for (int k = 0; k < 4; ++k)
#pragma unroll
          for (int b = 0; b < 4; ++b) {
            const unsigned int d = (words[k] >> (8 * b)) & 0xffu;
            const int bit = q * 16 + k * 4 + b;
            if (d & (KP1_DONE_TERMINATED | KP1_DONE_TRUNCATED)) {
              dmask |= 1ull << bit;
              if (d & KP1_DONE_SUCCESS) smask |= 1ull << bit;
            }
          }
      }
    } else {
      for (int b = 0; b < 64 && first + b < n; ++b) {
        const uint8_t d = dones[first + b];
        if (d & (KP1_DONE_TERMINATED | KP1_DONE_TRUNCATED)) {
          dmask |= 1ull << b;
          if (d & KP1_DONE_SUCCESS) smask |= 1ull << b;
        }
      }
    }
    unsigned long long busy = __ballot(dmask != 0ull);
    if (busy == 0ull) continue;
    c.ring_dirty = true;
    {
      int ended = __popcll(dmask);
      for (int off = 32; off > 0; off >>= 1) ended += __shfl_xor(ended, off);
      if (ended >= TRK_PARALLEL_MIN) {
        tracker_block_parallel(st, ring, c, ws, dmask, smask, ended);
        continue;
      }
    }
    int stage = c.stage, count = c.count, len = c.len, head = c.head, sum = c.sum, n_events = c.n_events;
    const int window = c.window;
    while (busy) {
      const int src = __ffsll((long long)busy) - 1;
      busy &= busy - 1;
      unsigned long long m = __shfl(dmask, src);
      const unsigned long long sm = __shfl(smask, src);
      if (lane != 0) continue;
      while (m) {
        const int b = __ffsll((long long)m) - 1;
        m &= m - 1;
        const int success = (int)((sm >> b) & 1ull);
        count += 1;
        if (len < window) {
          ring[head + len < window ? head + len : head + len - window] = success;
          len += 1;
          sum += success;
        } else {
          sum += success - ring[head];
          ring[head] = success;
          head = head + 1 < window ? head + 1 : 0;
        }
        if (stage >= c.max_stage) continue;
        if (count < c.min_episodes) continue;
        if (len < window) continue;
        const double rate = (double)sum / (double)len;
        if (rate >= c.threshold) {
          if (n_events < KP1_CURRICULUM_MAX_HISTORY) {
            kp1_curriculum_event& ev = st->events[n_events];
            ev.total_timesteps = c.timesteps;
            ev.from_stage = stage;
            ev.to_stage = stage + 1;
            ev.trigger_success_rate = rate;
          }
          n_events += 1;
          stage += 1;
          count = 0;
          len = 0;
          head = 0;
          sum = 0;
        }
      }
    }
    c.stage = __shfl(stage, 0); c.count = __shfl(count, 0); c.len = __shfl(len, 0); c.head = __shfl(head, 0);
    c.sum = __shfl(sum, 0); c.n_events = __shfl(n_events, 0);
  }
}

__global__ void __launch_bounds__(64) curriculum_kernel(kp1_curriculum_state* __restrict__ st, const uint8_t* __restrict__ dones, int n,
                                                        int steps_per_call) {
  __shared__ int ring[KP1_CURRICULUM_MAX_WINDOW];
  __shared__ uint8_t sbit[TRK_BLOCK];
  __shared__ uint16_t pfx[TRK_BLOCK + KP1_CURRICULUM_MAX_WINDOW + 1];
  const TrackerScratch ws = {sbit, pfx};
  {
    const int lane = threadIdx.x;
    bool any = false;
    for (int base = 0; base < n; base += 64 * 64) {
      const int first = base + lane * 64;
      if (first + 64 <= n && (reinterpret_cast<uintptr_t>(dones + first) & 15) == 0) {
        const uint4* p = reinterpret_cast<const uint4*>(dones + first);
        unsigned int acc = 0u;
#pragma unroll
        for (int q = 0; q < 4; ++q) {
          const uint4 w = p[q];
          acc |= w.x | w.y | w.z | w.w;
        }
        any |= (acc & (0x01010101u * (unsigned)(KP1_DONE_TERMINATED | KP1_DONE_TRUNCATED))) != 0u;
      } else {
        for (int b = 0; b < 64 && first + b < n; ++b) any |= (dones[first + b] & (KP1_DONE_TERMINATED | KP1_DONE_TRUNCATED)) != 0;
      }
    }
    if (__ballot(any) == 0ull) {
      if (lane == 0) atomicAdd(reinterpret_cast<unsigned long long*>(&st->num_timesteps), (unsigned long long)(long long)steps_per_call);
      return;
    }
  }
  TrackerCtx c;
  tracker_load(st, ring, c);
  curriculum_scan(st, ring, c, ws, dones, n, steps_per_call);
  tracker_store(st, ring, c);
}

__global__ void __launch_bounds__(64) curriculum_chunk_kernel(kp1_curriculum_state* __restrict__ st, const uint8_t* __restrict__ dones, int n_local,
                                                              int chunk_steps, int world, int steps_per_env_step) {
  __shared__ int ring[KP1_CURRICULUM_MAX_WINDOW];
  __shared__ uint8_t sbit[TRK_BLOCK];
  __shared__ uint16_t pfx[TRK_BLOCK + KP1_CURRICULUM_MAX_WINDOW + 1];
  const TrackerScratch ws = {sbit, pfx};
  TrackerCtx c;
  tracker_load(st, ring, c);
  for (int t = 0; t < chunk_steps; ++t)
    for (int r = 0; r < world; ++r)
      curriculum_scan(st, ring, c, ws, dones + ((int64_t)r * chunk_steps + t) * n_local, n_local, r == 0 ? steps_per_env_step : 0);
  tracker_store(st, ring, c);
}

__global__ void __launch_bounds__(64) curriculum_population_kernel(kp1_curriculum_state* __restrict__ states, const uint8_t* __restrict__ dones_all,
                                                                   int n, int steps_per_call) {
  __shared__ int ring[KP1_CURRICULUM_MAX_WINDOW];
  __shared__ uint8_t sbit[TRK_BLOCK];
  __shared__ uint16_t pfx[TRK_BLOCK + KP1_CURRICULUM_MAX_WINDOW + 1];
  const TrackerScratch ws = {sbit, pfx};
  kp1_curriculum_state* __restrict__ st = states + blockIdx.x;
  const uint8_t* __restrict__ dones = dones_all + (int64_t)blockIdx.x * n;
  {
    const int lane = threadIdx.x;
    bool any = false;
    for (int base = 0; base < n; base += 64 * 64) {
      const int first = base + lane * 64;
      if (first + 64 <= n && (reinterpret_cast<uintptr_t>(dones + first) & 15) == 0) {
        const uint4* p = reinterpret_cast<const uint4*>(dones + first);
        unsigned int acc = 0u;
#pragma unroll
        for (int q = 0; q < 4; ++q) {
          const uint4 w = p[q];
          acc |= w.x | w.y | w.z | w.w;
        }
        any |= (acc & (0x01010101u * (unsigned)(KP1_DONE_TERMINATED | KP1_DONE_TRUNCATED))) != 0u;
      } else {
        for (int b = 0; b < 64 && first + b < n; ++b) any |= (dones[first + b] & (KP1_DONE_TERMINATED | KP1_DONE_TRUNCATED)) != 0;
      }
    }
    if (__ballot(any) == 0ull) {
      if (lane == 0) atomicAdd(reinterpret_cast<unsigned long long*>(&st->num_timesteps), (unsigned long long)(long long)steps_per_call);
      return;
    }
  }
  TrackerCtx c;
  tracker_load(st, ring, c);
  curriculum_scan(st, ring, c, ws, dones, n, steps_per_call);
  tracker_store(st, ring, c);
}

int check_device(int device) {
  int count = 0;
  if (hipGetDeviceCount(&count) != hipSuccess || count <= 0) return fail(KP1_ERR_NO_DEVICE, "no HIP device: this library has no CPU path");
  if (device < 0 || device >= count) return fail(KP1_ERR_INVALID, "device index out of range");
  HIP_TRY(hipSetDevice(device));
  return KP1_OK;
}

}

extern "C" {

int kp1_gae_scan(int32_t device, const float* rewards, const float* values, const uint8_t* dones, const float* last_values, float gamma,
                 float gae_lambda, float* advantages, float* returns, int32_t T, int32_t N, void* stream) {
  if (!rewards || !values || !dones || !last_values || !advantages || !returns || T <= 0 || N <= 0) return fail(KP1_ERR_INVALID, "bad argument to kp1_gae_scan");
  int rc = check_device(device);
  if (rc != KP1_OK) return rc;
  const int block = N <= 16384 ? 64 : 256;
  hipLaunchKernelGGL(gae_scan_kernel, dim3((N + block - 1) / block), dim3(block), 0, (hipStream_t)stream, rewards, values, dones, last_values,
                     gamma, gae_lambda, advantages, returns, T, N);
  HIP_TRY(kp1::launch_status());
  return KP1_OK;
}

int kp1_gae_scan_replicas(int32_t device, const float* rewards, const float* values, const uint8_t* dones, const float* last_values,
                          const float* gamma_lambda, int32_t n_per_replica, float* advantages, float* returns, int32_t T, int32_t N, void* stream) {
  if (!rewards || !values || !dones || !last_values || !gamma_lambda || !advantages || !returns || T <= 0 || N <= 0)
    return fail(KP1_ERR_INVALID, "bad argument to kp1_gae_scan_replicas");
  if (n_per_replica <= 0 || N % n_per_replica != 0) return fail(KP1_ERR_INVALID, "kp1_gae_scan_replicas: N must be a multiple of n_per_replica");
  int rc = check_device(device);
  if (rc != KP1_OK) return rc;
  const int block = N <= 16384 ? 64 : 256;
  hipLaunchKernelGGL(gae_scan_replicas_kernel, dim3((N + block - 1) / block), dim3(block), 0, (hipStream_t)stream, rewards, values, dones,
                     last_values, gamma_lambda, n_per_replica, advantages, returns, T, N);
  HIP_TRY(kp1::launch_status());
  return KP1_OK;
}

}

namespace {
__global__ void __launch_bounds__(256) adv_minibatch_sums_kernel(const float* __restrict__ adv, const int64_t* __restrict__ idx, int64_t total, int64_t mb,
                                                                 double* __restrict__ out) {
  __shared__ double s1[256], s2[256];
  const int64_t begin = (int64_t)blockIdx.x * mb, end = begin + mb < total ? begin + mb : total;
  double a = 0.0, b = 0.0;
  for (int64_t i = begin + threadIdx.x; i < end; i += 256) {
    const double v = (double)adv[idx ? idx[i] : i];
    a += v;
    b += v * v;
  }
  s1[threadIdx.x] = a;
  s2[threadIdx.x] = b;
  __syncthreads();
  for (int k = 128; k > 0; k >>= 1) {
    if (threadIdx.x < k) {
      s1[threadIdx.x] += s1[threadIdx.x + k];
      s2[threadIdx.x] += s2[threadIdx.x + k];
    }
    __syncthreads();
  }
  if (threadIdx.x == 0) {
    out[3 * blockIdx.x] = s1[0];
    out[3 * blockIdx.x + 1] = s2[0];
    out[3 * blockIdx.x + 2] = (double)(end - begin);
  }
}
struct PermKeys { uint32_t mul[4], add[4]; };
__global__ void __launch_bounds__(256) permutation_kernel(int64_t* __restrict__ out, int64_t n, int bits, const PermKeys k) {
  const int64_t i = (int64_t)blockIdx.x * 256 + threadIdx.x;
  if (i >= n) return;
  const uint32_t mask = bits >= 32 ? 0xffffffffu : ((1u << bits) - 1u);
  const int sh = bits > 1 ? bits / 2 : 1;
  uint32_t x = (uint32_t)i;
  do {
#pragma unroll
    for (int r = 0; r < 4; ++r) {
      x = (x * k.mul[r] + k.add[r]) & mask;
      x ^= x >> sh;
    }
  } while ((int64_t)x >= n);
// ... 24 lines not shown
  while (((int64_t)1 << bits) < n) ++bits;
  PermKeys k;
  for (int r = 0; r < 4; ++r) {
    k.mul[r] = keys[r] | 1u;
    k.add[r] = keys[4 + r];
  }
  hipLaunchKernelGGL(permutation_kernel, dim3((unsigned)((n + 255) / 256)), dim3(256), 0, (hipStream_t)stream, out, n, bits, k);
  HIP_TRY(kp1::launch_status());
  return KP1_OK;
}

int kp1_adv_minibatch_stats(int32_t device, const double* sums, int64_t n_minibatches, float* out_stats, void* stream) {
  if (!sums || !out_stats || n_minibatches <= 0) return fail(KP1_ERR_INVALID, "bad argument to kp1_adv_minibatch_stats");
  int rc = check_device(device);
  if (rc != KP1_OK) return rc;
  hipLaunchKernelGGL(adv_minibatch_stats_kernel, dim3((unsigned)((n_minibatches + 63) / 64)), dim3(64), 0, (hipStream_t)stream, sums, n_minibatches,
                     out_stats);
  HIP_TRY(kp1::launch_status());
  return KP1_OK;
}

int kp1_adv_minibatch_sums(int32_t device, const float* advantages, const int64_t* idx, int64_t total, int64_t minibatch, double* out_sums,
                           void* stream) {
  if (!advantages || !out_sums || total <= 0 || minibatch <= 0) return fail(KP1_ERR_INVALID, "bad argument to kp1_adv_minibatch_sums");
  int rc = check_device(device);
  if (rc != KP1_OK) return rc;
  const int64_t n_mb = (total + minibatch - 1) / minibatch;
  hipLaunchKernelGGL(adv_minibatch_sums_kernel, dim3((unsigned)n_mb), dim3(256), 0, (hipStream_t)stream, advantages, idx, total, minibatch, out_sums);
  HIP_TRY(kp1::launch_status());
  return KP1_OK;
}

int kp1_bootstrap_truncated(int32_t device, float* rewards, const float* terminal_values, const uint8_t* dones, float gamma, int64_t count,
                            void* stream) {
  if (!rewards || !terminal_values || !dones || count <= 0) return fail(KP1_ERR_INVALID, "bad argument to kp1_bootstrap_truncated");
  int rc = check_device(device);
  if (rc != KP1_OK) return rc;
  hipLaunchKernelGGL(bootstrap_kernel, dim3((unsigned)((count + 255) / 256)), dim3(256), 0, (hipStream_t)stream, rewards, terminal_values, dones,
                     gamma, count);
  HIP_TRY(kp1::launch_status());
  return KP1_OK;
}

int kp1_curriculum_create(int32_t device, double success_rate_threshold, int32_t window_episodes, int32_t min_episodes_per_stage,
                          int32_t max_stage_index, int32_t initial_stage_index, kp1_curriculum_state** out_dev) {
  return kp1_curriculum_create_population(device, 1, success_rate_threshold, window_episodes, min_episodes_per_stage, max_stage_index,
                                          &initial_stage_index, out_dev);
}
int kp1_curriculum_create_population(int32_t device, int32_t n_replicas, double success_rate_threshold, int32_t window_episodes,
                                     int32_t min_episodes_per_stage, int32_t max_stage_index, const int32_t* initial_stages,
                                     kp1_curriculum_state** out_dev) {
  if (!out_dev || !initial_stages) return fail(KP1_ERR_INVALID, "NULL argument");
  if (n_replicas < 1 || n_replicas > KP1_CURRICULUM_MAX_REPLICAS) return fail(KP1_ERR_INVALID, "n_replicas must be in [1, KP1_CURRICULUM_MAX_REPLICAS]");
  int rc = check_device(device);
  if (rc != KP1_OK) return rc;
  std::vector<kp1_curriculum_state> h((size_t)n_replicas);
  for (int k = 0; k < n_replicas; ++k) {
    kp1_curriculum_state& s = h[(size_t)k];
    std::memset(&s, 0, sizeof s);
    s.success_rate_threshold = success_rate_threshold;
    s.window_episodes = window_episodes < 1 ? 1 : window_episodes;
    if (s.window_episodes > KP1_CURRICULUM_MAX_WINDOW) return fail(KP1_ERR_INVALID, "window_episodes exceeds KP1_CURRICULUM_MAX_WINDOW");
    s.min_episodes_per_stage = min_episodes_per_stage < 1 ? 1 : min_episodes_per_stage;
    s.max_stage_index = max_stage_index < 0 ? 0 : max_stage_index;
    int init = initial_stages[k] < s.max_stage_index ? initial_stages[k] : s.max_stage_index;
    s.stage_index = init < 0 ? 0 : init;
  }
  kp1_curriculum_state* d = nullptr;
  HIP_TRY(hipMalloc((void**)&d, sizeof(kp1_curriculum_state) * h.size()));
  HIP_TRY(hipMemcpy(d, h.data(), sizeof(kp1_curriculum_state) * h.size(), hipMemcpyHostToDevice));
  *out_dev = d;
  return KP1_OK;
}
int kp1_curriculum_destroy(int32_t device, kp1_curriculum_state* st_dev) {
  int rc = check_device(device);
  if (rc != KP1_OK) return rc;
  HIP_TRY(hipFree(st_dev));
  return KP1_OK;
}
int kp1_curriculum_observe(int32_t device, kp1_curriculum_state* st_dev, const uint8_t* dones, int32_t n, int32_t steps_per_call, void* stream) {
  if (!st_dev || !dones || n <= 0) return fail(KP1_ERR_INVALID, "bad argument to kp1_curriculum_observe");
  int rc = check_device(device);
  if (rc != KP1_OK) return rc;
  hipLaunchKernelGGL(curriculum_kernel, dim3(1), dim3(64), 0, (hipStream_t)stream, st_dev, dones, n, steps_per_call);
  HIP_TRY(kp1::launch_status());
  return KP1_OK;
}
int kp1_curriculum_observe_chunk(int32_t device, kp1_curriculum_state* st_dev, const uint8_t* dones, int32_t n_local, int32_t chunk_steps,
                                 int32_t world, void* stream) {
  if (!st_dev || !dones || n_local <= 0 || chunk_steps <= 0 || world <= 0) return fail(KP1_ERR_INVALID, "bad argument to kp1_curriculum_observe_chunk");
  int rc = check_device(device);
  if (rc != KP1_OK) return rc;
  hipLaunchKernelGGL(curriculum_chunk_kernel, dim3(1), dim3(64), 0, (hipStream_t)stream, st_dev, dones, n_local, chunk_steps, world, n_local * world);
  HIP_TRY(kp1::launch_status());
  return KP1_OK;
}
int kp1_curriculum_observe_population(int32_t device, kp1_curriculum_state* states_dev, const uint8_t* dones, int32_t n_per_replica,
                                      int32_t n_replicas, int32_t steps_per_call, void* stream) {
  if (!states_dev || !dones || n_per_replica <= 0 || n_replicas < 1 || n_replicas > KP1_CURRICULUM_MAX_REPLICAS)
    return fail(KP1_ERR_INVALID, "bad argument to kp1_curriculum_observe_population");
  int rc = check_device(device);
  if (rc != KP1_OK) return rc;
  hipLaunchKernelGGL(curriculum_population_kernel, dim3((unsigned)n_replicas), dim3(64), 0, (hipStream_t)stream, states_dev, dones, n_per_replica,
                     steps_per_call);
  HIP_TRY(kp1::launch_status());
  return KP1_OK;
}
int kp1_curriculum_read_replica(int32_t device, const kp1_curriculum_state* states_dev, int32_t n_replicas, int32_t k, kp1_curriculum_state* out_host,
                                void* stream) {
  if (!states_dev || !out_host) return fail(KP1_ERR_INVALID, "NULL argument");
  if (k < 0 || k >= n_replicas) return fail(KP1_ERR_INVALID, "replica index out of range");
  return kp1_curriculum_read(device, states_dev + k, out_host, stream);
}
int kp1_curriculum_read(int32_t device, const kp1_curriculum_state* st_dev, kp1_curriculum_state* out_host, void* stream) {
  if (!st_dev || !out_host) return fail(KP1_ERR_INVALID, "NULL argument");
  int rc = check_device(device);
  if (rc != KP1_OK) return rc;
  HIP_TRY(hipMemcpyAsync(out_host, st_dev, sizeof *out_host, hipMemcpyDeviceToHost, (hipStream_t)stream));
  HIP_TRY(hipStreamSynchronize((hipStream_t)stream));
  return KP1_OK;
}

}
```

### rl_brain_trainer_amd/curriculum.py

```python
from __future__ import annotations

import ctypes as C
from typing import Any, Sequence

import torch

from . import native

MAX_WINDOW = 1024
MAX_HISTORY = 64


class _Event(C.Structure):
    _fields_ = [("total_timesteps", C.c_int64), ("from_stage", C.c_int32), ("to_stage", C.c_int32), ("trigger_success_rate", C.c_double)]


class CurriculumState(C.Structure):
    _fields_ = [
        ("stage_index", C.c_int32), ("stage_episode_count", C.c_int32), ("ring_len", C.c_int32), ("ring_head", C.c_int32),
        ("window_episodes", C.c_int32), ("min_episodes_per_stage", C.c_int32), ("max_stage_index", C.c_int32), ("n_events", C.c_int32),
        ("success_rate_threshold", C.c_double), ("num_timesteps", C.c_int64),
        ("ring", C.c_int32 * MAX_WINDOW), ("events", _Event * MAX_HISTORY),
    ]


class PointCurriculum:
    def __init__(self, *, success_rate_threshold: float, window_episodes: int, min_episodes_per_stage: int, max_stage_index: int,
                 initial_stage_index: int = 0, device: torch.device | int = 0) -> None:
        self.L = native.load()
        self.device = torch.device("cuda", device) if isinstance(device, int) else torch.device(device)
        self._st = C.c_void_p()
        native.check(self.L.kp1_curriculum_create(self.device.index or 0, float(success_rate_threshold), int(window_episodes),
                                                  int(min_episodes_per_stage), int(max_stage_index), int(initial_stage_index), C.byref(self._st)))

    @property
    def stage_ptr(self) -> int:
        return int(self._st.value)

    def attach(self, env) -> None:
        native.check(self.L.kp1_bind_stage_ptr(env._handle, C.c_void_p(self.stage_ptr)))

    def observe(self, dones: torch.Tensor, steps_per_call: int) -> None:
        stream = torch.cuda.current_stream(self.device).cuda_stream
        native.check(self.L.kp1_curriculum_observe(self.device.index or 0, self._st, C.c_void_p(dones.data_ptr()), int(dones.numel()),
                                                   int(steps_per_call), C.c_void_p(stream)))

    def observe_chunk(self, dones_all: torch.Tensor, n_local: int, chunk_steps: int, world: int) -> None:
        assert dones_all.numel() == world * chunk_steps * n_local and dones_all.dtype == torch.uint8 and dones_all.is_contiguous()
        stream = torch.cuda.current_stream(self.device).cuda_stream
        native.check(self.L.kp1_curriculum_observe_chunk(self.device.index or 0, self._st, C.c_void_p(dones_all.data_ptr()), int(n_local), int(chunk_steps),
                                                         int(world), C.c_void_p(stream)))

    def read(self) -> CurriculumState:
        out = CurriculumState()
        stream = torch.cuda.current_stream(self.device).cuda_stream
        native.check(self.L.kp1_curriculum_read(self.device.index or 0, self._st, C.byref(out), C.c_void_p(stream)))
        return out

    def summary(self) -> dict[str, object]:
        return self._summary_of(self.read())

    @staticmethod
    def _summary_of(st: CurriculumState) -> dict[str, object]:
        n = st.ring_len
        recent = [st.ring[k] for k in range(n)]
        return {
            "stage_index": int(st.stage_index),
            "stage_episode_count": int(st.stage_episode_count),
            "recent_success_rate": float(sum(recent)) / float(n) if n else 0.0,
            "history": [
                {"from_stage_index": int(e.from_stage), "to_stage_index": int(e.to_stage),
                 "trigger_success_rate": float(e.trigger_success_rate), "total_timesteps": int(e.total_timesteps)}
                for e in list(st.events)[: min(st.n_events, MAX_HISTORY)]
            ],
        }

    def close(self) -> None:
        if self._st.value:
            self.L.kp1_curriculum_destroy(self.device.index or 0, self._st)
            self._st = C.c_void_p()


class PointCurriculumPopulation(PointCurriculum):

    def __init__(self, *, success_rate_threshold: float, window_episodes: int, min_episodes_per_stage: int, max_stage_index: int,
                 initial_stage_indices: Sequence[int], device: torch.device | int = 0) -> None:
        from .vec_env import MAX_REPLICAS

        stages = [int(s) for s in initial_stage_indices]
        if not 1 <= len(stages) <= MAX_REPLICAS:
            raise ValueError(f"PointCurriculumPopulation holds 1 to {MAX_REPLICAS} trackers (got {len(stages)} initial stages)")
        self.K = len(stages)
        self.env: Any = None
        self.L = native.load()
        self.device = torch.device("cuda", device) if isinstance(device, int) else torch.device(device)
        self._st = C.c_void_p()
        init = (C.c_int32 * self.K)(*stages)
        native.check(self.L.kp1_curriculum_create_population(self.device.index or 0, self.K, float(success_rate_threshold), int(window_episodes),
                                                             int(min_episodes_per_stage), int(max_stage_index), C.cast(init, C.c_void_p),
                                                             C.byref(self._st)))

    @property
    def stage_ptr(self) -> int:
        raise TypeError("a population tracker has one stage per replica: attach() binds all of them to a population env")

    def attach(self, env: Any) -> None:
        if not getattr(env, "is_population", False):
            raise TypeError("PointCurriculumPopulation tracks the replicas of an ArmKinematicPopulationVecEnv")
        if env.n_envs % self.K != 0 or getattr(env, "K", self.K) != self.K:
            raise ValueError(f"a population env of {env.n_envs} envs does not split into this tracker's {self.K} replicas")
        native.check(self.L.kp1_bind_population_stages(env._handle, C.c_void_p(self._st.value), self.K))
        env.launch_args_version += 1
        self.env = env

    def observe(self, dones: torch.Tensor, steps_per_call: int) -> None:
        if dones.numel() % self.K != 0 or dones.dtype != torch.uint8 or not dones.is_contiguous():
            raise ValueError(f"observe() takes the contiguous uint8 done bytes of all {self.K} replicas")
        stream = torch.cuda.current_stream(self.device).cuda_stream
        native.check(self.L.kp1_curriculum_observe_population(self.device.index or 0, self._st, C.c_void_p(dones.data_ptr()), dones.numel() // self.K,
                                                              self.K, int(steps_per_call), C.c_void_p(stream)))

    def observe_chunk(self, dones_all: torch.Tensor, n_local: int, chunk_steps: int, world: int) -> None:
        raise TypeError("the population tracker has no data-parallel form")

    def read(self, k: int = 0) -> CurriculumState:
        out = CurriculumState()
        stream = torch.cuda.current_stream(self.device).cuda_stream
        native.check(self.L.kp1_curriculum_read_replica(self.device.index or 0, self._st, self.K, int(k), C.byref(out), C.c_void_p(stream)))
# ... 28 lines not shown
```

### rl_brain_trainer_amd/mlp.py

```python
from __future__ import annotations

import ctypes as C

import torch

from . import native

OBS_DIM, OBS_PAD, ACT_DIM = 56, 64, 7


def _p(t: torch.Tensor | None):
    return C.c_void_p(t.data_ptr()) if t is not None else None


class MlpKernels:
    def __init__(self, hidden: int, device: torch.device, max_batch: int = 8192, obs_dim: int = OBS_DIM, replicas: int = 1) -> None:
        self.L = native.load()
        L = self.L
        vp, i32, f32 = C.c_void_p, C.c_int32, C.c_float
        L.kp1_mlp_create_ex.argtypes = [i32, i32, i32, i32, C.POINTER(vp)]
        L.kp1_mlp_create_population.argtypes = [i32, i32, i32, i32, i32, C.POINTER(vp)]
        L.kp1_mlp_replicas.argtypes = [vp]
        L.kp1_mlp_replicas.restype = i32
        L.kp1_mlp_destroy.argtypes = [vp]
        L.kp1_mlp_num_params_ex.argtypes = [i32, i32]
        L.kp1_mlp_num_params_ex.restype = C.c_int64
        L.kp1_mlp_pack_weights.argtypes = [vp, vp, vp]
        L.kp1_mlp_forward.argtypes = [vp, vp, i32, i32, vp, vp, vp, vp, vp, vp, vp]
        L.kp1_mlp_forward_env_step.argtypes = [vp, vp, vp, i32, vp, vp, vp, vp, vp, vp, vp, vp, vp]
        L.kp1_mlp_loss_grad.argtypes = [vp, vp, i32, vp, i32, vp, vp, vp, vp, f32, f32, vp, f32, f32, f32, f32, vp, vp, i32, vp]
        L.kp1_mlp_adam_step.argtypes = [vp, vp, vp, vp, vp, f32, f32, f32, i32, i32, vp]
        L.kp1_mlp_time_kernels.argtypes = [vp, vp, i32, i32, i32, vp, vp, vp]
        L.kp1_mlp_placement_check.argtypes = [i32, i32, vp, vp]
        L.kp1_mlp_set_option.argtypes = [vp, i32, i32]
        L.kp1_mlp_profile_read.argtypes = [vp, vp, vp]
        L.kp1_mlp_set_replica_hparams.argtypes = [vp, vp, i32, vp]
        self.hidden = hidden
        self.device = device
        self.max_batch = int(max_batch)
        self._h = vp()
        self.obs_dim = int(obs_dim)
        self.obs_pad = 64 if self.obs_dim <= 64 else 128
        if replicas == 1:
            native.check(L.kp1_mlp_create_ex(device.index or 0, hidden, self.obs_dim, self.max_batch, C.byref(self._h)))
        else:
            native.check(L.kp1_mlp_create_population(device.index or 0, hidden, self.obs_dim, self.max_batch, int(replicas), C.byref(self._h)))
        self.replicas = int(L.kp1_mlp_replicas(self._h))
        self.num_params = int(L.kp1_mlp_num_params_ex(hidden, self.obs_dim))

    def close(self) -> None:
        if self._h.value:
            self.L.kp1_mlp_destroy(self._h)
            self._h = C.c_void_p()

    OPT_FUSED = 1

    def set_fused(self, on: bool) -> None:
        native.check(self.L.kp1_mlp_set_option(self._h, self.OPT_FUSED, int(bool(on))))

    OPT_ACTOR_EXTRA_STEPS = 2

    def set_actor_extra_steps(self, steps: int) -> None:
        native.check(self.L.kp1_mlp_set_option(self._h, self.OPT_ACTOR_EXTRA_STEPS, int(steps)))

    OPT_STEP_COUNT = 3

    def set_step_count(self, steps: int) -> None:
        native.check(self.L.kp1_mlp_set_option(self._h, self.OPT_STEP_COUNT, int(steps)))

    OPT_BF16X3_WGRAD = 5

    def set_bf16x3_wgrad(self, on: bool) -> None:
        native.check(self.L.kp1_mlp_set_option(self._h, self.OPT_BF16X3_WGRAD, int(bool(on))))

    OPT_PROFILE = 4
    PROFILE_SLOTS = ("mlp_train_tile", "gemm_tn_split", "grad_finalize", "adam")

    def set_profile(self, on: bool) -> None:
        native.check(self.L.kp1_mlp_set_option(self._h, self.OPT_PROFILE, int(bool(on))))

    def profile_read(self) -> dict[str, dict[str, float]]:
        us = (C.c_float * 4)()
        cnt = (C.c_int32 * 4)()
        native.check(self.L.kp1_mlp_profile_read(self._h, C.cast(us, C.c_void_p), C.cast(cnt, C.c_void_p)))
        return {name: {"us": float(us[i]), "launches": int(cnt[i])} for i, name in enumerate(self.PROFILE_SLOTS)}

    HPARAM_FIELDS = ("learning_rate", "adam_eps", "max_grad_norm", "clip_range", "ent_coef", "vf_coef")

    def set_replica_hparams(self, rows: list[dict[str, float]] | None) -> None:
        if rows is None:
            native.check(self.L.kp1_mlp_set_replica_hparams(self._h, None, 0, self._stream()))
            return
        table = (C.c_float * (len(rows) * len(self.HPARAM_FIELDS)))(*[float(r[f]) for r in rows for f in self.HPARAM_FIELDS])
        native.check(self.L.kp1_mlp_set_replica_hparams(self._h, C.cast(table, C.c_void_p), len(rows), self._stream()))

    def _stream(self):
        return C.c_void_p(torch.cuda.current_stream(self.device).cuda_stream)

    def pack(self, flat_params: torch.Tensor) -> None:
        assert flat_params.numel() == self.replicas * self.num_params and flat_params.dtype == torch.float32 and flat_params.is_contiguous()
        native.check(self.L.kp1_mlp_pack_weights(self._h, _p(flat_params), self._stream()))

    def forward(self, obs: torch.Tensor, *, noise=None, mean=None, value=None, action=None, clipped=None, log_prob=None) -> None:
        assert obs.shape[0] % self.replicas == 0
        n, stride = obs.shape[0] // self.replicas, obs.shape[1]
        assert obs.is_contiguous() and obs.dtype == torch.float32
        native.check(self.L.kp1_mlp_forward(self._h, _p(obs), stride, n, _p(noise), _p(mean), _p(value), _p(action), _p(clipped), _p(log_prob), self._stream()))

    def forward_env_step(self, env, obs: torch.Tensor, *, noise, value, action, log_prob, next_obs, reward, done, terminal_obs) -> None:
        assert obs.is_contiguous() and obs.dtype == torch.float32 and obs.shape[0] == env.n_envs
        native.check(self.L.kp1_mlp_forward_env_step(self._h, env._handle, _p(obs), obs.shape[1], _p(noise), _p(value), _p(action), _p(log_prob),
                                                     _p(next_obs), _p(reward), _p(done), _p(terminal_obs), self._stream()))

    def mean_value(self, obs: torch.Tensor) -> tuple[torch.Tensor, torch.Tensor]:
        n = obs.shape[0]
        mean = torch.empty((n, ACT_DIM), dtype=torch.float32, device=obs.device)
        value = torch.empty(n, dtype=torch.float32, device=obs.device)
        for s in range(0, n, self.max_batch):
            e = min(s + self.max_batch, n)
            self.forward(obs[s:e], mean=mean[s:e], value=value[s:e])
        return mean, value

    def loss_grad(self, obs: torch.Tensor, idx: torch.Tensor | None, n: int, actions, old_logp, adv, ret, *, clip_range: float, ent_coef: float,
                  vf_coef: float, inv_count: float, grad_out: torch.Tensor, stats_out: torch.Tensor | None, adv_stats: torch.Tensor | None = None,
                  normalize: bool = True, grad_is_zero: bool = False) -> None:
        assert obs.is_contiguous() and grad_out.numel() == self.replicas * self.num_params
        assert self.replicas == 1 or (idx is not None and idx.numel() == self.replicas * n)
        inv_std = 0.0 if normalize else -1.0
        native.check(self.L.kp1_mlp_loss_grad(self._h, _p(obs), obs.shape[-1], _p(idx), n, _p(actions), _p(old_logp), _p(adv), _p(ret), 0.0, inv_std,
                                              _p(adv_stats), clip_range, ent_coef, vf_coef, inv_count, _p(grad_out), _p(stats_out), int(grad_is_zero), self._stream()))

    def adam_step(self, params, grad, exp_avg, exp_avg_sq, *, lr: float, eps: float, max_grad_norm: float, step: int,
                  fused_norm: bool = False) -> None:
        native.check(self.L.kp1_mlp_adam_step(self._h, _p(params), _p(grad), _p(exp_avg), _p(exp_avg_sq), lr, eps, max_grad_norm, step,
                                              2 if fused_norm else 0, self._stream()))

    def placement_check(self, n_rows: int) -> dict[str, int | float]:
        out = (C.c_int32 * 8)()
        native.check(self.L.kp1_mlp_placement_check(self.device.index or 0, int(n_rows), C.cast(out, C.c_void_p), self._stream()))
        wgs, pairs, same, rr, cus, used, arrived, xcds = (int(v) for v in out)
        return {"workgroups": wgs, "compute_units": cus, "compute_units_used": used, "second_tile_on_same_cu": same, "second_tile_pairs": pairs,
                "on_xcd_of_block_index_mod_8": rr, "xcds_among_first_8_blocks": xcds, "all_resident": arrived == wgs}

    def time_kernels(self, obs: torch.Tensor, n: int, iters: int = 20) -> dict[str, dict[str, float]]:
        ms = (C.c_float * 6)()
        fl = (C.c_double * 6)()
        native.check(self.L.kp1_mlp_time_kernels(self._h, _p(obs), obs.shape[-1], n, iters, C.cast(ms, C.c_void_p), C.cast(fl, C.c_void_p), self._stream()))
        names = ("gemm_nt_fwd_l2", "gemm_nt_bwd_dz1", "gemm_tn_dw2", "gemm_nt_fwd_l1", "mlp_train_tile", "gemm_tn_split")
        return {nm: {"ms": float(ms[i]), "flops": float(fl[i]), "tflops": float(fl[i]) / (float(ms[i]) * 1e-3) / 1e12}
                for i, nm in enumerate(names) if ms[i] > 0}
```

### rl_brain_trainer_amd/native.py

```python
from __future__ import annotations

import ctypes as C
import re
from pathlib import Path

from . import config as kcfg

PKG_DIR = Path(__file__).resolve().parent
LIB_PATH = PKG_DIR / "libkp1.so"

KP1_OK = 0
REAL_F32, REAL_F64 = 0, 1
DONE_TERMINATED, DONE_TRUNCATED, DONE_SUCCESS, DONE_INVALID = 1, 2, 4, 8
FLAG_PRE_NEAR_HIT, FLAG_NEAR_HIT, FLAG_SUCCESS = 1, 2, 4


class EvalBuffers(C.Structure):
    _fields_ = [(n, C.c_void_p) for n in ("metrics", "counters", "flags", "state", "hand_metrics", "hand_step", "hand_success", "hand_state", "n_alive")]


class Kp1Error(RuntimeError):
    pass


_lib: C.CDLL | None = None


def declared_symbols() -> list[str]:
    names: list[str] = []
    for header in sorted((kcfg.repo_root() / "include").glob("*.h")):
        text = re.sub(r"/\*.*?\*/", "", header.read_text(), flags=re.S)
        names += re.findall(r"\b(kp1_[a-z0-9_]+)\s*\(", text)
    seen, out = set(), []
    for n in names:
        if n not in seen and not n.endswith("_t"):
            seen.add(n)
            out.append(n)
    return out


def load() -> C.CDLL:
    global _lib
    if _lib is not None:
        return _lib
    if not LIB_PATH.exists():
        raise Kp1Error(
            f"{LIB_PATH} is missing: the HIP extension has not been built. There is no CPU fallback; "
            "build it with `python -c 'import __graft_entry__ as g; g.build()'`."
        )
    L = C.CDLL(str(LIB_PATH))
    vp, i32, u64, i64 = C.c_void_p, C.c_int32, C.c_uint64, C.c_int64
    L.kp1_last_error.restype = C.c_char_p
    L.kp1_abi_version.restype = C.c_int
    L.kp1_config_size.restype = u64
    L.kp1_config_default.argtypes = [C.POINTER(kcfg.Kp1Config)]
    L.kp1_create.argtypes = [C.POINTER(kcfg.Kp1Config), i32, i32, i32, u64, u64, vp, C.POINTER(vp)]
    L.kp1_destroy.argtypes = [vp]
    L.kp1_set_stream.argtypes = [vp, vp]
    L.kp1_num_envs.argtypes = [vp]
    L.kp1_set_stage.argtypes = [vp, i32]
    L.kp1_get_stage.argtypes = [vp, C.POINTER(i32)]
    L.kp1_set_mode.argtypes = [vp, i32]
    L.kp1_update_config.argtypes = [vp, C.POINTER(kcfg.Kp1Config)]
    L.kp1_set_handoff_states.argtypes = [vp, vp, i32]
    L.kp1_seed.argtypes = [vp, u64, u64]
    L.kp1_reset.argtypes = [vp, vp, C.POINTER(kcfg.ResetOpts), vp]
    L.kp1_step.argtypes = [vp, vp, vp, vp, vp, vp, i32]
    L.kp1_observe.argtypes = [vp, vp]
    L.kp1_get_info.argtypes = [vp, C.POINTER(kcfg.InfoView)]
    L.kp1_eval_accumulate.argtypes = [vp, C.POINTER(EvalBuffers), vp, vp, vp, i32, vp, i32, vp]
    L.kp1_get_reward_components.argtypes = [vp, C.POINTER(vp), C.POINTER(i32)]
    L.kp1_enable_reward_components.argtypes = [vp, i32]
    L.kp1_component_name.argtypes = [i32, i32]
    L.kp1_component_name.restype = C.c_char_p
    L.kp1_num_components.argtypes = [i32]
    L.kp1_get_state.argtypes = [vp] + [vp] * 5
    L.kp1_set_state.argtypes = [vp] + [vp] * 5 + [i32]
    L.kp1_rng_get.argtypes = [vp, vp]
    L.kp1_rng_set.argtypes = [vp, vp]
    L.kp1_state_snapshot.argtypes = [vp]
    L.kp1_state_restore.argtypes = [vp]
    L.kp1_fk_pose6.argtypes = [i32, i32, vp, vp, i64, vp]
    L.kp1_pose_error.argtypes = [i32, i32, vp, vp, vp, vp, vp, i64, vp]
    L.kp1_joint_utils.argtypes = [i32, i32, C.POINTER(kcfg.Kp1Config), vp, vp, vp, vp, vp, vp, i64, vp]
    L.kp1_rng_seed_state.argtypes = [u64, C.POINTER(kcfg.RngState)]
    f32 = C.c_float
    L.kp1_gae_scan.argtypes = [i32, vp, vp, vp, vp, f32, f32, vp, vp, i32, i32, vp]
    L.kp1_gae_scan_replicas.argtypes = [i32, vp, vp, vp, vp, vp, i32, vp, vp, i32, i32, vp]
    L.kp1_bootstrap_truncated.argtypes = [i32, vp, vp, vp, f32, i64, vp]
    L.kp1_adv_minibatch_sums.argtypes = [i32, vp, vp, i64, i64, vp, vp]
    L.kp1_adv_minibatch_stats.argtypes = [i32, vp, i64, vp, vp]
    L.kp1_random_permutation.argtypes = [i32, i64, vp, vp, vp]
    L.kp1_curriculum_create.argtypes = [i32, C.c_double, i32, i32, i32, i32, C.POINTER(vp)]
    L.kp1_curriculum_destroy.argtypes = [i32, vp]
    L.kp1_curriculum_observe.argtypes = [i32, vp, vp, i32, i32, vp]
    L.kp1_curriculum_observe_chunk.argtypes = [i32, vp, vp, i32, i32, i32, vp]
    L.kp1_curriculum_read.argtypes = [i32, vp, vp, vp]
    L.kp1_bind_stage_ptr.argtypes = [vp, vp]
    L.kp1_curriculum_create_population.argtypes = [i32, i32, C.c_double, i32, i32, i32, vp, C.POINTER(vp)]
    L.kp1_curriculum_observe_population.argtypes = [i32, vp, vp, i32, i32, i32, vp]
    L.kp1_curriculum_read_replica.argtypes = [i32, vp, i32, i32, vp, vp]
    L.kp1_bind_population_stages.argtypes = [vp, vp, i32]
    L.kp1_seed_blocks.argtypes = [vp, vp, i32, i32]
    L.kp1_set_obs_stride.argtypes = [vp, i32]
    if L.kp1_config_size() != C.sizeof(kcfg.Kp1Config):
        raise Kp1Error(f"kp1_config layout mismatch: library {L.kp1_config_size()} vs binding {C.sizeof(kcfg.Kp1Config)}")
    _lib = L
    return L


def check(rc: int) -> None:
    if rc != KP1_OK:
        msg = load().kp1_last_error().decode(errors="replace")
        if rc == -1:
            raise ValueError(msg)
        raise Kp1Error(f"kp1 error {rc}: {msg}")


def component_names(mode: int) -> list[str]:
    L = load()
    return [L.kp1_component_name(mode, i).decode() for i in range(L.kp1_num_components(mode))]
```

### rl_brain_trainer_amd/ppo.py

```python
from __future__ import annotations

import ctypes as C
import math
import os
import time
from dataclasses import dataclass, field
from typing import Any

import numpy as np
import torch

from . import config as kcfg
from . import native
from .curriculum import PointCurriculum
from .vec_env import ArmKinematicVecEnv

OBS_DIM = kcfg.OBS_DIM
ACT_DIM = kcfg.NJ


@dataclass
class PPOConfig:

    learning_rate: float = 3e-4
# ... 307 lines not shown
            self.dist.all_reduce(captured, op=self.dist.ReduceOp.MIN)
            good = bool(captured.item() > 0.5)
            if good:
                buf.fill_(float(self.rank + 1))
                gathered.zero_()
                g.replay()
                torch.cuda.synchronize(device)
                want = torch.arange(1, self.world_size + 1, dtype=torch.uint8, device=device)[:, None].expand(-1, 16)
                good = bool(torch.all(buf == expect).item()) and bool(torch.equal(gathered, want))
            dog.cancel()
            verdict.fill_(1.0 if good else 0.0)
        self.dist.all_reduce(verdict, op=self.dist.ReduceOp.MIN)
        return bool(verdict.item() > 0.5)


def _bind_policy(policy: ActorCritic, flat: torch.Tensor) -> None:
    flat.copy_(policy.flat)
    policy.flat = flat
    off = 0
    for name, shape in policy.spec:
        n = math.prod(shape)
        policy.views[name] = flat[off:off + n].view(shape)
        off += n


def load_adam_state(opt: dict[str, Any], spec, adam_m: torch.Tensor, adam_v: torch.Tensor) -> tuple[int, int]:
    steps, off = [], 0
    for i, (name, shape) in enumerate(spec):
        n = math.prod(shape)
        st = opt["state"].get(i)
        if st is None or tuple(st["exp_avg"].shape) != tuple(shape):
            raise ValueError(f"optimizer state of parameter {i} ({name}) does not match the policy")
        adam_m[off:off + n].copy_(st["exp_avg"].to(adam_m.device, torch.float32).reshape(-1))
        adam_v[off:off + n].copy_(st["exp_avg_sq"].to(adam_v.device, torch.float32).reshape(-1))
        steps.append((name, int(float(st["step"]))))
        off += n
    actor = [s_ for n_, s_ in steps if n_.startswith(("mlp_extractor.policy_net", "action_net"))]
    rest = [s_ for n_, s_ in steps if not n_.startswith(("mlp_extractor.policy_net", "action_net"))]
    if len(set(actor)) != 1 or len(set(rest)) != 1 or actor[0] < rest[0]:
        raise ValueError(f"unsupported per-tensor Adam step pattern {steps}")
    return rest[0], actor[0] - rest[0]


def restore_saved_hyperparameters(cfg: "PPOConfig", data: dict[str, Any]) -> dict[str, Any]:
    taken = {}
    for key, cast in (("gamma", float), ("gae_lambda", float), ("ent_coef", float), ("vf_coef", float), ("max_grad_norm", float),
                      ("n_epochs", int), ("normalize_advantage", bool)):
        v = data.get(key)
        if isinstance(v, (int, float, bool)) and not (isinstance(v, bool) and cast is not bool):
            setattr(cfg, key, cast(v))
            taken[key] = cast(v)
    clip = data.get("clip_range")
    if isinstance(clip, dict) and isinstance(clip.get("value"), (int, float)):
        cfg.clip_range = float(clip["value"])
        taken["clip_range"] = cfg.clip_range
    return taken


class PPO:

    def __init__(self, env: ArmKinematicVecEnv, cfg: PPOConfig, *, curriculum: PointCurriculum | None = None,
                 dist: Dist | None = None, backend: str = "hip", use_graphs: bool = True) -> None:
        if backend != "hip":
            raise ValueError("backend must be 'hip': the HIP kernels are the only training path")
        if getattr(env, "is_population", False):
            raise TypeError("PPO trains one seed; a population env (K replicas in one handle) is trained by population.ApproachPopulationPPO")
        if env.dtype != torch.float32:
            raise ValueError("PPO drives the production f32 env")
        self.env = env
        self.curriculum = curriculum
        self._setup(cfg, [cfg.seed], [env], [curriculum], dist or Dist(), use_graphs, min_batch=8192, stacked=False)
        self.policy = self.policies[0]
        T, N, dev = cfg.n_steps, self.n_envs, self.device
        self.done_chunk = 1
        if self.dist.enabled:
            self.done_chunk = math.gcd(T, max(int(os.environ.get("KP1_DONE_EXCHANGE_STEPS", "16")), 1))
            self._done_gather = torch.zeros((self.dist.world_size, self.done_chunk, N), dtype=torch.uint8, device=dev)
            self._record_stage = None
            if curriculum is not None and getattr(curriculum, "needs_episode_records", False):
                self._record_stage = torch.zeros((self.done_chunk, N), dtype=torch.uint8, device=dev)
        self._fused_env_step = bool(type(env) is ArmKinematicVecEnv and env.dtype == torch.float32 and cfg.hidden == 256
                                    and self.obs_dim <= 64 and not getattr(env, "_reward_components_on", False)
                                    and os.environ.get("KP1_FUSED_ROLLOUT", "1") != "0")

    def _setup(self, cfg: PPOConfig, seeds: list[int], envs: list[Any], curricula: list[Any], dist: Dist, use_graphs: bool, *,
               min_batch: int, stacked: bool) -> None:
        self.cfg = cfg
        self.dist = dist
        self.backend = "hip"
        self.L = native.load()
        self.K = K = len(seeds)
        self.envs, self.curricula = envs, curricula
        self.device = dev = envs[0].device
        self.n_envs = N = envs[0].n_envs
        self.obs_dim = int(getattr(envs[0], "obs_dim", OBS_DIM))
        self.obs_w = 64 if self.obs_dim <= 64 else 128
        for env, cur in zip(envs, curricula):
            if cur is not None:
                cur.attach(env)
            env.set_obs_stride(self.obs_w)
        self.policies = [ActorCritic(cfg.hidden, dev, seed=s, obs_dim=self.obs_dim) for s in seeds]
        self.flat = self.policies[0].flat
        if stacked:
            self.flat = torch.zeros((K, self.policies[0].numel), dtype=torch.float32, device=dev)
            for k, pol in enumerate(self.policies):
                _bind_policy(pol, self.flat[k])
        self.dist.broadcast(self.flat)
        self.adam_m = torch.zeros_like(self.flat)
        self.adam_v = torch.zeros_like(self.flat)
        self.grad = torch.zeros_like(self.flat)
        self.stats_dev = torch.zeros((K, 4), dtype=torch.float32, device=dev)
        self.adam_t = 0
        self.n_train_calls = 0
        self.actor_extra_steps = 0
        self.num_timesteps = 0
        T, KN = cfg.n_steps, K * N
        self.obs_buf = torch.zeros((T + 1, KN, self.obs_w), dtype=torch.float32, device=dev)
        self.term_obs_buf = torch.zeros((T, KN, self.obs_w), dtype=torch.float32, device=dev)
        self.act_buf = torch.zeros((T, KN, ACT_DIM), dtype=torch.float32, device=dev)
        self.clip_act = torch.zeros((KN, ACT_DIM), dtype=torch.float32, device=dev)
        self.logp_buf = torch.zeros((T, KN), dtype=torch.float32, device=dev)
        self.val_buf = torch.zeros((T, KN), dtype=torch.float32, device=dev)
        self.rew_buf = torch.zeros((T, KN), dtype=torch.float32, device=dev)
        self.done_buf = torch.zeros((T, KN), dtype=torch.uint8, device=dev)
        self.adv_buf = torch.zeros((T, KN), dtype=torch.float32, device=dev)
        self.ret_buf = torch.zeros((T, KN), dtype=torch.float32, device=dev)
        self.noise_all = torch.zeros((T, KN, ACT_DIM), dtype=torch.float32, device=dev)
        self.perm = torch.zeros((K, T * N), dtype=torch.int64, device=dev)
        self.gens = [torch.Generator(device=dev).manual_seed(int(s) + 7919 * self.dist.rank) for s in seeds]
        self._perm_rngs = [np.random.Generator(np.random.PCG64(np.random.SeedSequence([int(s), self.dist.rank, 0x6B7031]))) for s in seeds]
        self._needs_reset = True
        self._last_stats_dev: tuple[torch.Tensor, int] | None = None
        self._last_stats_host: list[dict[str, float]] = [{} for _ in range(K)]
        from . import mlp as _mlp

        local_bs = max(cfg.batch_size // self.dist.world_size, 1)
        self._mlp = _mlp.MlpKernels(cfg.hidden, dev, max_batch=max(N, local_bs, min_batch), obs_dim=self.obs_dim, replicas=K)
        self._mlp.pack(self.flat)
        if os.environ.get("KP1_BF16X3_WGRAD", "0") == "1" and cfg.hidden == 256:
            self._mlp.set_bf16x3_wgrad(True)
        self.use_graphs = bool(use_graphs)
        self.dist.use_stream_collectives(dev)
        self.graph_mode = self.dist.graph_mode(dev) if self.use_graphs else "none"
        self._first_replay_checked = {"rollout": not (self.dist.enabled and self.graph_mode == "captured"),
                                      "epoch": not (self.dist.enabled and self.graph_mode == "captured")}
        self._rollout_graph = None
        self._epoch_graph = None
        self._epoch_policy = os.environ.get("KP1_DP_EPOCH", "auto")
        self._epoch_auto = None
        self.epoch_form = "one graph" if self.graph_mode == "captured" else ("eager launches" if self.graph_mode == "none" or self._epoch_policy == "eager" else "graph segments")
        self._rollout_graph_key = None
        self._epoch_graph_key = None
        self._epoch_warm = False
        self._kernels_warm = False
        self.step_callback = None

    def _sl(self, k: int) -> slice:
        return slice(k * self.n_envs, (k + 1) * self.n_envs)

    PERM_CIPHER_MIN = 1 << 17

    def _draw_perm(self, k: int) -> None:
        out = self.perm[k]
        total = out.numel()
        if total < self.PERM_CIPHER_MIN:
            torch.randperm(total, device=self.device, generator=self.gens[k], out=out)
# ... 54 lines not shown
                    raise RuntimeError("restore_hyperparameters must happen before the first update")
                restored["hyperparameters"] = restore_saved_hyperparameters(self.cfg, data)
        return restored

    def _forward(self, obs: torch.Tensor) -> tuple[torch.Tensor, torch.Tensor]:
        return self._mlp.mean_value(obs.contiguous())

    def predict(self, obs: torch.Tensor, deterministic: bool = True) -> torch.Tensor:
        with torch.no_grad():
            mean, _ = self._forward(obs)
            if not deterministic:
                mean = mean + torch.exp(self.policy.views["log_std"]) * torch.randn(mean.shape, device=mean.device, generator=self.gens[0])
            return mean.clamp(-1.0, 1.0)

    def predict_unclipped(self, obs: torch.Tensor) -> torch.Tensor:
        with torch.no_grad():
            return self._forward(obs)[0]

    def _bootstrap_truncated(self, dense: bool = False) -> None:
        cfg, env = self.cfg, self.env
        T, N = cfg.n_steps, self.n_envs
        stream = torch.cuda.current_stream(self.device).cuda_stream
        dev = self.device.index or 0
        if not dense:
            max_steps = max(int(env.config.c.termination.max_episode_steps), 1)
            cap = min(N * (T // max_steps + 1), T * N)
            trunc = (self.done_buf.view(-1) & 3) == 2
            idx = torch.nonzero_static(trunc, size=cap, fill_value=0).view(-1)
            valid = torch.arange(cap, device=self.device) < trunc.sum()
            sel = self.term_obs_buf.view(T * N, self.obs_w).index_select(0, idx)
            tv = torch.empty(cap, dtype=torch.float32, device=self.device)
            for s0 in range(0, cap, self._mlp.max_batch):
                e0 = min(s0 + self._mlp.max_batch, cap)
                self._mlp.forward(sel[s0:e0], value=tv[s0:e0])
            self.rew_buf.view(-1).index_add_(0, idx, torch.where(valid, cfg.gamma * tv, torch.zeros_like(tv)))
        else:
            _, tv = self._forward(self.term_obs_buf.view(T * N, self.obs_w))
            tv = tv.contiguous()
            native.check(self.L.kp1_bootstrap_truncated(dev, C.c_void_p(self.rew_buf.data_ptr()), C.c_void_p(tv.data_ptr()),
                                                        C.c_void_p(self.done_buf.data_ptr()), cfg.gamma, T * N, C.c_void_p(stream)))

    @torch.no_grad()
    def collect_rollouts(self) -> None:
        cfg = self.cfg
        T, N = cfg.n_steps, self.n_envs
        if self._needs_reset:
            self._reset_envs()
            self._needs_reset = False
        else:
            self.obs_buf[0].copy_(self.obs_buf[T])
        world = self.dist.world_size
        graph_rollout = self.use_graphs and self.step_callback is None
        self._draw_noise()
        if graph_rollout:
            key = (tuple(getattr(env, "launch_args_version", 0) for env in self.envs), tuple(cur is not None for cur in self.curricula),
                   cfg.gamma, cfg.gae_lambda)
            if self._rollout_graph is None or self._rollout_graph_key != key:
                self._capture_rollout()
                self._rollout_graph_key = key
            self._replay_checked("rollout", self._rollout_graph)
        for t in range(0 if not graph_rollout else T, T):
            self._rollout_step_hip(t)
            if self.step_callback is not None:
                self.step_callback(self.done_buf[t])
        if not graph_rollout:
            self._kernels_warm = True
        self.num_timesteps += T * N * world
        if not graph_rollout:
            self._post_rollout()

    def _post_rollout(self) -> None:
        cfg = self.cfg
        T, KN = cfg.n_steps, self.K * self.n_envs
        self._bootstrap_truncated()
        stream = torch.cuda.current_stream(self.device).cuda_stream
        dev = self.device.index or 0
        last_v = torch.empty(KN, dtype=torch.float32, device=self.device)
        self._mlp.forward(self.obs_buf[T], value=last_v)
        native.check(self.L.kp1_gae_scan(dev, C.c_void_p(self.rew_buf.data_ptr()), C.c_void_p(self.val_buf.data_ptr()),
                                         C.c_void_p(self.done_buf.data_ptr()), C.c_void_p(last_v.data_ptr()), cfg.gamma, cfg.gae_lambda,
                                         C.c_void_p(self.adv_buf.data_ptr()), C.c_void_p(self.ret_buf.data_ptr()), T, KN, C.c_void_p(stream)))

    def _rollout_step_hip(self, t: int) -> None:
        self._policy_env_step(t)
        self._curriculum_observe(t)

    def _policy_env_step(self, t: int) -> None:
        if self._fused_env_step:
            self._mlp.forward_env_step(self.env, self.obs_buf[t], noise=self.noise_all[t], value=self.val_buf[t], action=self.act_buf[t],
                                       log_prob=self.logp_buf[t], next_obs=self.obs_buf[t + 1], reward=self.rew_buf[t], done=self.done_buf[t],
                                       terminal_obs=self.term_obs_buf[t])
        else:
            self._mlp.forward(self.obs_buf[t], noise=self.noise_all[t], value=self.val_buf[t], action=self.act_buf[t],
                              clipped=self.clip_act, log_prob=self.logp_buf[t])
            self.env.step_into(self.clip_act, self.obs_buf[t + 1], self.rew_buf[t], self.done_buf[t], self.term_obs_buf[t], True)

    def _capture_rollout(self) -> None:
        T = self.cfg.n_steps
        if not self._kernels_warm:
            side = torch.cuda.Stream(device=self.device)
            side.wait_stream(torch.cuda.current_stream(self.device))
            with torch.cuda.stream(side):
                for env in self.envs:
                    env.use_current_stream()
                    if hasattr(env, "snapshot"):
                        env.snapshot()
                self._policy_env_step(0)
                self._warm_curricula()
                self._post_rollout()
                fresh = []
                for k, env in enumerate(self.envs):
                    env.use_current_stream()
                    if hasattr(env, "snapshot"):
                        env.restore()
                    else:
                        fresh.append(k)
                if fresh:
                    self._reset_envs(fresh)
            torch.cuda.current_stream(self.device).wait_stream(side)
            self._kernels_warm = True
        torch.cuda.synchronize(self.device)

        def body() -> None:
            for t in range(T):
                self._rollout_step_hip(t)
            self._post_rollout()

        self._rollout_graph = self._capture(body, on_begin=self._envs_use_current_stream)
        self._envs_use_current_stream()

    def _reset_envs(self, which: list[int] | None = None) -> None:
        for k in range(len(self.envs)) if which is None else which:
            self.obs_buf[0, self._sl(k)].copy_(self.envs[k].reset())

    def _warm_curricula(self) -> None:
        for k, cur in enumerate(self.curricula):
            if cur is not None:
                cur.observe(self.done_buf[0, self._sl(k)].zero_(), 0)

    def _envs_use_current_stream(self) -> None:
        for env in self.envs:
            env.use_current_stream()

    def _capture(self, body, on_begin=None):
        if self.dist.enabled and self.graph_mode == "segmented":
            seg = GraphSegments(self.device, on_begin=on_begin)
            self.dist._segments = seg
            try:
                seg.begin()
                body()
                seg.finish()
            except BaseException:
                seg.abort()
                raise
            finally:
                self.dist._segments = None
            return seg
        g = torch.cuda.CUDAGraph()
        with torch.cuda.graph(g, capture_error_mode="thread_local" if self.dist.enabled else "global"):
            if on_begin is not None:
                on_begin()
            body()
        return g

    def _replay_checked(self, what: str, graph) -> None:
        if self._first_replay_checked[what]:
            graph.replay()
            return
        dog = self.dist.watchdog(300.0, f"the first replay of the {what} graph with captured RCCL collectives")
        graph.replay()
        torch.cuda.synchronize(self.device)
        ok = self.dist.ranks_agree(self.policy.flat)
        dog.cancel()
        self._first_replay_checked[what] = True
# ... 211 lines not shown
```

Before: 11.40 million.

## Fold curriculum tracker update into the fused policy+env rollout kernel

Removes the separate per-step curriculum_kernel launch in approach mode. Each block of the fused forward/env-step kernel now runs the tracker update for the previous step's dones on a spare wave. Reset lanes spin-wait on an LDS slot for the folded stage, and tracker state ping-pongs between two device buffers; a closing observe runs after the last step. This saves one launch per rollout step, at the cost of redundant per-block tracker work, an intra-block spin dependency, and a cap on env count.

```diff
diff --git a/include/kp1_ppo.h b/include/kp1_ppo.h
--- a/include/kp1_ppo.h
+++ b/include/kp1_ppo.h
@@ -49,6 +49,8 @@
 int kp1_curriculum_observe_chunk(int32_t device, kp1_curriculum_state* st_dev, const uint8_t* dones, int32_t n_local, int32_t chunk_steps,
                                  int32_t world, void* stream);
 int kp1_curriculum_read(int32_t device, const kp1_curriculum_state* st_dev, kp1_curriculum_state* out_host, void* stream);
+int kp1_curriculum_observe_from(int32_t device, const kp1_curriculum_state* st_in_dev, kp1_curriculum_state* st_out_dev, const uint8_t* dones,
+                                int32_t n, int32_t steps_per_call, void* stream);
 int kp1_bind_stage_ptr(kp1_env* env, const int32_t* stage_dev);
 
 #define KP1_CURRICULUM_MAX_REPLICAS 16
@@ -124,8 +126,16 @@
 int kp1_mlp_forward(kp1_mlp* m, const float* obs, int32_t obs_stride, int32_t n, const float* noise, float* mean, float* value,
                     float* action, float* clipped_action, float* log_prob, void* stream);
 
+typedef struct kp1_tracker_fold {
+  const kp1_curriculum_state* state_in;
+  kp1_curriculum_state* state_out;
+  const uint8_t* prev_dones;
+  int32_t steps_per_call;
+} kp1_tracker_fold;
+
 int kp1_mlp_forward_env_step(kp1_mlp* m, kp1_env* env, const float* obs, int32_t obs_stride, const float* noise, float* value, float* action,
-                             float* log_prob, float* next_obs, float* reward, uint8_t* done, float* terminal_obs, void* stream);
+                             float* log_prob, float* next_obs, float* reward, uint8_t* done, float* terminal_obs, void* stream,
+                             const kp1_tracker_fold* tracker);
 
 int kp1_mlp_loss_grad(kp1_mlp* m, const float* obs, int32_t obs_stride, const int64_t* idx, int32_t n, const float* actions,
                       const float* old_log_prob, const float* advantages, const float* returns, float adv_mean, float adv_inv_std,
diff --git a/rl_brain_trainer_amd/csrc/kp1_env_step.inc b/rl_brain_trainer_amd/csrc/kp1_env_step.inc
--- a/rl_brain_trainer_amd/csrc/kp1_env_step.inc
+++ b/rl_brain_trainer_amd/csrc/kp1_env_step.inc
@@ -304,8 +304,18 @@
   const kp1_dock_curriculum_stage* pop_dock;
 };
 
+__device__ __forceinline__ int wait_folded_stage(const int* slot) {
+  for (unsigned polls = 0; polls < (1u << 24); ++polls) {
+    const int v = __hip_atomic_load(slot, __ATOMIC_RELAXED, __HIP_MEMORY_SCOPE_WORKGROUP);
+    if (v != 0) return v - 1;
+    __builtin_amdgcn_s_sleep(2);
+  }
+  __builtin_trap();
+  return 0;
+}
 template <typename R, int MODE, bool COMPS, bool POP = false>
-__device__ __forceinline__ void step_env_lane(const StepArgs<R>& a, const int64_t i, const R* __restrict__ act_src, float* __restrict__ o) {
+__device__ __forceinline__ void step_env_lane(const StepArgs<R>& a, const int64_t i, const R* __restrict__ act_src, float* __restrict__ o,
+                                              const int* folded_stage = nullptr) {
   const int64_t n = a.st.n;
   KP1_ETR(0)
   const DevCfg<R>& __restrict__ cfg = *scalar_cache_warm(a.cfg);
@@ -458,7 +468,7 @@
     int stage = a.stage_index;
     const DevSampler& smp = uniform_block(a.smp);
     if constexpr (POP && !LIVE) stage = kp_clipi(a.pop_states[(uint32_t)i / (uint32_t)a.n_per_replica].stage_index, 0, kp_maxi(smp.n_stages - 1, 0));
-    else if (a.stage_ptr) stage = kp_clipi(*a.stage_ptr, 0, kp_maxi(smp.n_stages - 1, 0));
+    else if (a.stage_ptr) stage = kp_clipi(folded_stage ? wait_folded_stage(folded_stage) : *a.stage_ptr, 0, kp_maxi(smp.n_stages - 1, 0));
     reset_env<R, MODE, LIVE>(st, cfg, smp, a.handoff, none, stage, i, o, live);
     st.r(F_POS_ERR, i) = curr_pos;
     st.r(F_ORI_ERR, i) = curr_ori;
diff --git a/rl_brain_trainer_amd/csrc/kp1_mlp.hip b/rl_brain_trainer_amd/csrc/kp1_mlp.hip
--- a/rl_brain_trainer_amd/csrc/kp1_mlp.hip
+++ b/rl_brain_trainer_amd/csrc/kp1_mlp.hip
@@ -1080,6 +1080,7 @@
 }
 
 #include "kp1_env_step.inc"
+#include "kp1_tracker.inc"
 #include "kp1_mlp_tile.inc"
 #include "kp1_mlp_fused.inc"
 
@@ -1586,7 +1587,8 @@
 }
 
 int kp1_mlp_forward_env_step(kp1_mlp* m, kp1_env* env, const float* obs, int32_t obs_stride, const float* noise, float* value, float* action,
-                             float* log_prob, float* next_obs, float* reward, uint8_t* done, float* terminal_obs, void* stream) {
+                             float* log_prob, float* next_obs, float* reward, uint8_t* done, float* terminal_obs, void* stream,
+                             const kp1_tracker_fold* tracker) {
   if (!m || !env || !obs || !action || !next_obs || !reward || !done) return fail(KP1_ERR_INVALID, "NULL argument to kp1_mlp_forward_env_step");
   if (m->K > 1) return fail(KP1_ERR_UNSUPPORTED, "kp1_mlp_forward_env_step is not available on population handles");
   if (!(m->fused && m->Hp == FU_HP) || m->L.INP != 64)
@@ -1604,6 +1606,15 @@
   fa.obs = obs; fa.obs_stride = obs_stride; fa.Kreal = obs_stride >= m->L.INP ? m->L.INP : m->L.IN; fa.inp = m->L.INP; fa.idx = nullptr; fa.n = (int)n_envs;
   fa.k = m->k;
   fa.noise = noise; fa.value = value; fa.action = action; fa.log_prob = log_prob;
+  if (tracker && tracker->prev_dones) {
+    if (mode != KP1_MODE_APPROACH) return fail(KP1_ERR_UNSUPPORTED, "kp1_mlp_forward_env_step carries the PointCurriculum tracker in approach mode only");
+    if (!tracker->state_in || !tracker->state_out || tracker->state_in == tracker->state_out)
+      return fail(KP1_ERR_INVALID, "kp1_tracker_fold needs two different tracker states");
+    if (tracker->prev_dones == done) return fail(KP1_ERR_INVALID, "kp1_tracker_fold: prev_dones is the buffer this step writes");
+    if (fa.env.stage_ptr && fa.env.stage_ptr != &tracker->state_in->stage_index && fa.env.stage_ptr != &tracker->state_out->stage_index)
+      return fail(KP1_ERR_INVALID, "kp1_tracker_fold: the env handle follows another tracker's stage (kp1_bind_stage_ptr)");
+    fa.trk_in = tracker->state_in; fa.trk_out = tracker->state_out; fa.trk_dones = tracker->prev_dones; fa.trk_steps = tracker->steps_per_call;
+  }
   rc = launch_fused_infer_env(fa, mode, (hipStream_t)stream);
   if (rc != KP1_OK) return rc;
   HIP_TRY(kp1::launch_status());
diff --git a/rl_brain_trainer_amd/csrc/kp1_mlp_tile.inc b/rl_brain_trainer_amd/csrc/kp1_mlp_tile.inc
--- a/rl_brain_trainer_amd/csrc/kp1_mlp_tile.inc
+++ b/rl_brain_trainer_amd/csrc/kp1_mlp_tile.inc
@@ -16,6 +16,7 @@
   int stagger_ticks, n_cus;
   StepArgs<float> env;
   unsigned short* sp_h1; unsigned short* sp_dz2; unsigned short* sp_dz1; unsigned short* sp_xf; int64_t sp_plane, sp_plane_x;
+  const kp1_curriculum_state* trk_in; kp1_curriculum_state* trk_out; const uint8_t* trk_dones; int trk_steps;
 };
 
 typedef __bf16 bf16x8 __attribute__((ext_vector_type(8)));
@@ -55,6 +56,7 @@
 constexpr int FU_SCRATCH = 4 * FU_BM * 8 + FU_BM * 8 + FU_NW * 24 + 64;
 constexpr int FU_LDS_FLOATS = 2 * FU_BM * FU_AP + HEADS * FU_HP + FU_SCRATCH;
 static_assert(FU_LDS_FLOATS * 4 * 2 <= 160 * 1024, "the two training tiles of one CU must fit its LDS");
+static_assert(TRK_LDS_BYTES <= FU_BM * FU_AP * 4 && (FU_BM * FU_AP * 4) % 16 == 0, "the folded tracker's window and scratch live in bufB");
 
 template <bool TRAIN, int K1S, int ENV = 0, bool SPLIT = false>
 __global__ void __launch_bounds__(FU_NTH, ENV ? 1 : 2) mlp_tile_kernel(const FusedArgs a) {
@@ -237,6 +239,8 @@
       misc[1] = inv_std;
     }
   }
+  int* const trk_slot = reinterpret_cast<int*>(misc + 8);
+  if (ENV == 1 && tid == 0) *trk_slot = 0;
   float bias1[CB], bias2[CB];
 #pragma unroll
   for (int c = 0; c < CB; ++c) {
@@ -346,8 +350,17 @@
         if (wave == 0) {
           const bool live = lane < BM && m0 + lane < a.n;
           float o[KP1_OBS_DIM];
-          if (live) step_env_lane<float, ENV == 1 ? KP1_MODE_APPROACH : KP1_MODE_DOCK, false>(a.env, (int64_t)(m0 + lane), dout + lane * 8, o);
+          const int* const folded = (ENV == 1 && a.trk_dones != nullptr) ? trk_slot : nullptr;
+          if (live) step_env_lane<float, ENV == 1 ? KP1_MODE_APPROACH : KP1_MODE_DOCK, false>(a.env, (int64_t)(m0 + lane), dout + lane * 8, o, folded);
           store_obs_tile(a.env.obs, (int64_t)m0, min(BM, a.n - m0), o, live, a.env.obs_stride, bufA);
+        }
+        if constexpr (ENV == 1) {
+          if (wave == 1 && a.trk_dones != nullptr) {
+            tracker_observe_wave(a.trk_in, a.trk_out, blockIdx.x == 0, tracker_fetch(a.trk_dones, a.n, lane), a.trk_dones, a.n, a.trk_steps, lane, reinterpret_cast<char*>(bufB),
+                                 [&](int stage) {
+                                   if (lane == 0) __hip_atomic_store(trk_slot, stage + 1, __ATOMIC_RELAXED, __HIP_MEMORY_SCOPE_WORKGROUP);
+                                 });
+          }
         }
       }
     } else if (l_ok && l_out == 7 && a.value) {
diff --git a/rl_brain_trainer_amd/csrc/kp1_ppo.hip b/rl_brain_trainer_amd/csrc/kp1_ppo.hip
--- a/rl_brain_trainer_amd/csrc/kp1_ppo.hip
+++ b/rl_brain_trainer_amd/csrc/kp1_ppo.hip
@@ -59,320 +59,37 @@
   if ((d & KP1_DONE_TRUNCATED) && !(d & KP1_DONE_TERMINATED)) rewards[k] += gamma * tv[k];
 }
 
-struct TrackerCtx {
-  int stage, count, len, head, window, min_episodes, max_stage, n_events, sum;
-  double threshold;
-  long long timesteps;
-  bool ring_dirty;
-};
-
-__device__ __forceinline__ void tracker_load(const kp1_curriculum_state* __restrict__ st, int* __restrict__ ring, TrackerCtx& c) {
+#include "kp1_tracker.inc"
+
+__global__ void __launch_bounds__(64) curriculum_kernel(const kp1_curriculum_state* st_in, kp1_curriculum_state* st_out, const uint8_t* __restrict__ dones,
+                                                        int n, int steps_per_call) {
+  __shared__ __attribute__((aligned(16))) char trk_lds[TRK_LDS_BYTES];
   const int lane = threadIdx.x;
-  c.stage = st->stage_index; c.count = st->stage_episode_count; c.len = st->ring_len; c.head = st->ring_head;
-  c.window = st->window_episodes; c.min_episodes = st->min_episodes_per_stage; c.max_stage = st->max_stage_index; c.n_events = st->n_events;
-  c.threshold = st->success_rate_threshold; c.timesteps = st->num_timesteps;
-  c.ring_dirty = false;
-  int part = 0;
-  for (int k = lane; k < c.window; k += 64) {
-    const int v = st->ring[k];
-    ring[k] = v;
-    const int age = k >= c.head ? k - c.head : k - c.head + c.window;
-    if (age < c.len) part += v;
-  }
-  for (int off = 32; off > 0; off >>= 1) part += __shfl_xor(part, off);
-  c.sum = part;
-  __syncthreads();
-}
-
-__device__ __forceinline__ void tracker_store(kp1_curriculum_state* __restrict__ st, const int* __restrict__ ring, const TrackerCtx& c) {
-  const int lane = threadIdx.x;
-  __syncthreads();
-  if (c.ring_dirty)
-    for (int k = lane; k < c.window; k += 64) st->ring[k] = ring[k];
-  if (lane == 0) {
-    st->stage_index = c.stage; st->stage_episode_count = c.count; st->ring_len = c.len; st->ring_head = c.head;
-    st->n_events = c.n_events; st->num_timesteps = c.timesteps;
-  }
-}
-
-constexpr int TRK_BLOCK = 64 * 64, TRK_PARALLEL_MIN = 192;
-struct TrackerScratch { uint8_t* sbit; uint16_t* pfx; };
-
-__device__ __forceinline__ void tracker_append_run(int* __restrict__ ring, TrackerCtx& c, const uint8_t* __restrict__ sbit, int pos, int R) {
-  const int lane = threadIdx.x, W = c.window;
-  const int j0 = R > W ? R - W : 0;
-  __syncthreads();
-  for (int j = j0 + lane; j < R; j += 64) ring[(c.head + c.len + j) % W] = sbit[pos + j];
-  __syncthreads();
-  const int over = c.len + R - W;
-  c.head = over > 0 ? (c.head + over) % W : c.head;
-  c.len = c.len + R < W ? c.len + R : W;
-  c.count += R;
-  int part = 0;
-  for (int k = lane; k < W; k += 64) {
-    const int age = k >= c.head ? k - c.head : k - c.head + W;
-    if (age < c.len) part += ring[k];
-  }
-  for (int off = 32; off > 0; off >>= 1) part += __shfl_xor(part, off);
-  c.sum = part;
-}
-
-__device__ __forceinline__ void tracker_block_parallel(kp1_curriculum_state* __restrict__ st, int* __restrict__ ring, TrackerCtx& c, const TrackerScratch& ws,
-                                                       unsigned long long dmask, unsigned long long smask, int E) {
-  const int lane = threadIdx.x, W = c.window;
-  int mine = __popcll(dmask), off = mine;
-  for (int d = 1; d < 64; d <<= 1) {
-    const int up = __shfl_up(off, d);
-    if (lane >= d) off += up;
-  }
-  off -= mine;
-  __syncthreads();
-  for (unsigned long long m = dmask; m; m &= m - 1) {
-    const int b = __ffsll((long long)m) - 1;
-    ws.sbit[off++] = (uint8_t)((smask >> b) & 1ull);
-  }
-  __syncthreads();
-  int pos = 0;
-  while (pos < E) {
-    const int R = E - pos;
-    if (c.stage >= c.max_stage) {
-      tracker_append_run(ring, c, ws.sbit, pos, R);
-      break;
-    }
-    const int L = c.len, T = L + R;
-    const int seg = (T + 63) / 64, j_lo = lane * seg < T ? lane * seg : T, j_hi = j_lo + seg < T ? j_lo + seg : T;
-    auto y = [&](int j) -> int { return j < L ? ring[(c.head + j) % W] : (int)ws.sbit[pos + (j - L)]; };
-    int tot = 0;
-    for (int j = j_lo; j < j_hi; ++j) tot += y(j);
-    int run = tot;
-    for (int d = 1; d < 64; d <<= 1) {
-      const int up = __shfl_up(run, d);
-      if (lane >= d) run += up;
-    }
-    run -= tot;
-    __syncthreads();
-    if (lane == 0) ws.pfx[0] = 0;
-    for (int j = j_lo; j < j_hi; ++j) {
-      run += y(j);
-      ws.pfx[j + 1] = (uint16_t)run;
-    }
-    __syncthreads();
-    int best = R;
-    for (int r = lane; r < R; r += 64) {
-      const int filled = L + r + 1;
-      if (filled < W || c.count + r + 1 < c.min_episodes) continue;
-      const int wsum = (int)ws.pfx[filled] - (int)ws.pfx[filled - W];
-      if ((double)wsum / (double)W >= c.threshold) {
-        best = r;
-        break;
-      }
-    }
-    for (int d = 32; d > 0; d >>= 1) {
-      const int o = __shfl_xor(best, d);
-      best = o < best ? o : best;
-    }
-    if (best >= R) {
-      tracker_append_run(ring, c, ws.sbit, pos, R);
-      break;
-    }
-    const int filled = L + best + 1;
-    const double rate = (double)((int)ws.pfx[filled] - (int)ws.pfx[filled - W]) / (double)W;
-    if (lane == 0 && c.n_events < KP1_CURRICULUM_MAX_HISTORY) {
-      kp1_curriculum_event& ev = st->events[c.n_events];
-      ev.total_timesteps = c.timesteps;
-      ev.from_stage = c.stage;
-      ev.to_stage = c.stage + 1;
-      ev.trigger_success_rate = rate;
-    }
-    c.n_events += 1;
-    c.stage += 1;
-    c.count = 0;
-    c.len = 0;
-    c.head = 0;
-    c.sum = 0;
-    pos += best + 1;
-  }
-}
-
-__device__ __forceinline__ void curriculum_scan(kp1_curriculum_state* __restrict__ st, int* __restrict__ ring, TrackerCtx& c, const TrackerScratch& ws,
-                                                const uint8_t* __restrict__ dones, int n, int steps_per_call) {
-  const int lane = threadIdx.x;
-  c.timesteps += steps_per_call;
-  for (int base = 0; base < n; base += 64 * 64) {
-    const int first = base + lane * 64;
-    unsigned long long dmask = 0ull, smask = 0ull;
-    if (first + 64 <= n && (reinterpret_cast<uintptr_t>(dones + first) & 15) == 0) {
-      const uint4* p = reinterpret_cast<const uint4*>(dones + first);
-      uint4 w[4];
-#pragma unroll
-      for (int q = 0; q < 4; ++q) w[q] = p[q];
-#pragma unroll
-      for (int q = 0; q < 4; ++q) {
-        const unsigned int words[4] = {w[q].x, w[q].y, w[q].z, w[q].w};
-#pragma unroll
-        for (int k = 0; k < 4; ++k)
-#pragma unroll
-          for (int b = 0; b < 4; ++b) {
-            const unsigned int d = (words[k] >> (8 * b)) & 0xffu;
-            const int bit = q * 16 + k * 4 + b;
-            if (d & (KP1_DONE_TERMINATED | KP1_DONE_TRUNCATED)) {
-              dmask |= 1ull << bit;
-              if (d & KP1_DONE_SUCCESS) smask |= 1ull << bit;
-            }
-          }
-      }
-    } else {
-      for (int b = 0; b < 64 && first + b < n; ++b) {
-        const uint8_t d = dones[first + b];
-        if (d & (KP1_DONE_TERMINATED | KP1_DONE_TRUNCATED)) {
-          dmask |= 1ull << b;
-          if (d & KP1_DONE_SUCCESS) smask |= 1ull << b;
-        }
-      }
-    }
-    unsigned long long busy = __ballot(dmask != 0ull);
-    if (busy == 0ull) continue;
-    c.ring_dirty = true;
-    {
-      int ended = __popcll(dmask);
-      for (int off = 32; off > 0; off >>= 1) ended += __shfl_xor(ended, off);
-      if (ended >= TRK_PARALLEL_MIN) {
-        tracker_block_parallel(st, ring, c, ws, dmask, smask, ended);
-        continue;
-      }
-    }
-    int stage = c.stage, count = c.count, len = c.len, head = c.head, sum = c.sum, n_events = c.n_events;
-    const int window = c.window;
-    while (busy) {
-      const int src = __ffsll((long long)busy) - 1;
-      busy &= busy - 1;
-      unsigned long long m = __shfl(dmask, src);
-      const unsigned long long sm = __shfl(smask, src);
-      if (lane != 0) continue;
-      while (m) {
-        const int b = __ffsll((long long)m) - 1;
-        m &= m - 1;
-        const int success = (int)((sm >> b) & 1ull);
-        count += 1;
-        if (len < window) {
-          ring[head + len < window ? head + len : head + len - window] = success;
-          len += 1;
-          sum += success;
-        } else {
-          sum += success - ring[head];
-          ring[head] = success;
-          head = head + 1 < window ? head + 1 : 0;
-        }
-        if (stage >= c.max_stage) continue;
-        if (count < c.min_episodes) continue;
-        if (len < window) continue;
-        const double rate = (double)sum / (double)len;
-        if (rate >= c.threshold) {
-          if (n_events < KP1_CURRICULUM_MAX_HISTORY) {
-            kp1_curriculum_event& ev = st->events[n_events];
-            ev.total_timesteps = c.timesteps;
-            ev.from_stage = stage;
-            ev.to_stage = stage + 1;
-            ev.trigger_success_rate = rate;
-          }
-          n_events += 1;
-          stage += 1;
-          count = 0;
-          len = 0;
-          head = 0;
-          sum = 0;
-        }
-      }
-    }
-    c.stage = __shfl(stage, 0); c.count = __shfl(count, 0); c.len = __shfl(len, 0); c.head = __shfl(head, 0);
-    c.sum = __shfl(sum, 0); c.n_events = __shfl(n_events, 0);
-  }
-}
-
-__global__ void __launch_bounds__(64) curriculum_kernel(kp1_curriculum_state* __restrict__ st, const uint8_t* __restrict__ dones, int n,
-                                                        int steps_per_call) {
-  __shared__ int ring[KP1_CURRICULUM_MAX_WINDOW];
-  __shared__ uint8_t sbit[TRK_BLOCK];
-  __shared__ uint16_t pfx[TRK_BLOCK + KP1_CURRICULUM_MAX_WINDOW + 1];
-  const TrackerScratch ws = {sbit, pfx};
-  {
-    const int lane = threadIdx.x;
-    bool any = false;
-    for (int base = 0; base < n; base += 64 * 64) {
-      const int first = base + lane * 64;
-      if (first + 64 <= n && (reinterpret_cast<uintptr_t>(dones + first) & 15) == 0) {
-        const uint4* p = reinterpret_cast<const uint4*>(dones + first);
-        unsigned int acc = 0u;
-#pragma unroll
-        for (int q = 0; q < 4; ++q) {
-          const uint4 w = p[q];
-          acc |= w.x | w.y | w.z | w.w;
-        }
-        any |= (acc & (0x01010101u * (unsigned)(KP1_DONE_TERMINATED | KP1_DONE_TRUNCATED))) != 0u;
-      } else {
-        for (int b = 0; b < 64 && first + b < n; ++b) any |= (dones[first + b] & (KP1_DONE_TERMINATED | KP1_DONE_TRUNCATED)) != 0;
-      }
-    }
-    if (__ballot(any) == 0ull) {
-      if (lane == 0) atomicAdd(reinterpret_cast<unsigned long long*>(&st->num_timesteps), (unsigned long long)(long long)steps_per_call);
-      return;
-    }
-  }
-  TrackerCtx c;
-  tracker_load(st, ring, c);
-  curriculum_scan(st, ring, c, ws, dones, n, steps_per_call);
-  tracker_store(st, ring, c);
+  tracker_observe_wave(st_in, st_out, true, tracker_fetch(dones, n, lane), dones, n, steps_per_call, lane, trk_lds, [](int) {});
 }
 
 __global__ void __launch_bounds__(64) curriculum_chunk_kernel(kp1_curriculum_state* __restrict__ st, const uint8_t* __restrict__ dones, int n_local,
                                                               int chunk_steps, int world, int steps_per_env_step) {
-  __shared__ int ring[KP1_CURRICULUM_MAX_WINDOW];
-  __shared__ uint8_t sbit[TRK_BLOCK];
-  __shared__ uint16_t pfx[TRK_BLOCK + KP1_CURRICULUM_MAX_WINDOW + 1];
-  const TrackerScratch ws = {sbit, pfx};
+  __shared__ __attribute__((aligned(16))) char trk_lds[TRK_LDS_BYTES];
+  int* ring = reinterpret_cast<int*>(trk_lds);
+  const TrackerScratch ws = {reinterpret_cast<uint8_t*>(trk_lds + TRK_LDS_RING), reinterpret_cast<uint16_t*>(trk_lds + TRK_LDS_RING + TRK_LDS_SBIT)};
+  const TrackerEvents evs = {st->events, nullptr};
+  const int lane = threadIdx.x;
   TrackerCtx c;
-  tracker_load(st, ring, c);
+  tracker_load(st, ring, c, lane);
   for (int t = 0; t < chunk_steps; ++t)
     for (int r = 0; r < world; ++r)
-      curriculum_scan(st, ring, c, ws, dones + ((int64_t)r * chunk_steps + t) * n_local, n_local, r == 0 ? steps_per_env_step : 0);
-  tracker_store(st, ring, c);
+      curriculum_scan(evs, ring, c, ws, dones + ((int64_t)r * chunk_steps + t) * n_local, n_local, r == 0 ? steps_per_env_step : 0, lane);
+  tracker_store(st, ring, c, lane, false);
 }
 
 __global__ void __launch_bounds__(64) curriculum_population_kernel(kp1_curriculum_state* __restrict__ states, const uint8_t* __restrict__ dones_all,
                                                                    int n, int steps_per_call) {
-  __shared__ int ring[KP1_CURRICULUM_MAX_WINDOW];
-  __shared__ uint8_t sbit[TRK_BLOCK];
-  __shared__ uint16_t pfx[TRK_BLOCK + KP1_CURRICULUM_MAX_WINDOW + 1];
-  const TrackerScratch ws = {sbit, pfx};
-  kp1_curriculum_state* __restrict__ st = states + blockIdx.x;
+  __shared__ __attribute__((aligned(16))) char trk_lds[TRK_LDS_BYTES];
+  kp1_curriculum_state* st = states + blockIdx.x;
   const uint8_t* __restrict__ dones = dones_all + (int64_t)blockIdx.x * n;
-  {
-    const int lane = threadIdx.x;
-    bool any = false;
-    for (int base = 0; base < n; base += 64 * 64) {
-      const int first = base + lane * 64;
-      if (first + 64 <= n && (reinterpret_cast<uintptr_t>(dones + first) & 15) == 0) {
-        const uint4* p = reinterpret_cast<const uint4*>(dones + first);
-        unsigned int acc = 0u;
-#pragma unroll
-        for (int q = 0; q < 4; ++q) {
-          const uint4 w = p[q];
-          acc |= w.x | w.y | w.z | w.w;
-        }
-        any |= (acc & (0x01010101u * (unsigned)(KP1_DONE_TERMINATED | KP1_DONE_TRUNCATED))) != 0u;
-      } else {
-        for (int b = 0; b < 64 && first + b < n; ++b) any |= (dones[first + b] & (KP1_DONE_TERMINATED | KP1_DONE_TRUNCATED)) != 0;
-      }
-    }
-    if (__ballot(any) == 0ull) {
-      if (lane == 0) atomicAdd(reinterpret_cast<unsigned long long*>(&st->num_timesteps), (unsigned long long)(long long)steps_per_call);
-      return;
-    }
-  }
-  TrackerCtx c;
-  tracker_load(st, ring, c);
-  curriculum_scan(st, ring, c, ws, dones, n, steps_per_call);
-  tracker_store(st, ring, c);
+  const int lane = threadIdx.x;
+  tracker_observe_wave(st, st, true, tracker_fetch(dones, n, lane), dones, n, steps_per_call, lane, trk_lds, [](int) {});
 }
 
 int check_device(int device) {
@@ -563,7 +280,16 @@
   if (!st_dev || !dones || n <= 0) return fail(KP1_ERR_INVALID, "bad argument to kp1_curriculum_observe");
   int rc = check_device(device);
   if (rc != KP1_OK) return rc;
-  hipLaunchKernelGGL(curriculum_kernel, dim3(1), dim3(64), 0, (hipStream_t)stream, st_dev, dones, n, steps_per_call);
+  hipLaunchKernelGGL(curriculum_kernel, dim3(1), dim3(64), 0, (hipStream_t)stream, (const kp1_curriculum_state*)st_dev, st_dev, dones, n, steps_per_call);
+  HIP_TRY(kp1::launch_status());
+  return KP1_OK;
+}
+int kp1_curriculum_observe_from(int32_t device, const kp1_curriculum_state* st_in_dev, kp1_curriculum_state* st_out_dev, const uint8_t* dones, int32_t n,
+                                int32_t steps_per_call, void* stream) {
+  if (!st_in_dev || !st_out_dev || !dones || n <= 0) return fail(KP1_ERR_INVALID, "bad argument to kp1_curriculum_observe_from");
+  int rc = check_device(device);
+  if (rc != KP1_OK) return rc;
+  hipLaunchKernelGGL(curriculum_kernel, dim3(1), dim3(64), 0, (hipStream_t)stream, st_in_dev, st_out_dev, dones, n, steps_per_call);
   HIP_TRY(kp1::launch_status());
   return KP1_OK;
 }
diff --git a/rl_brain_trainer_amd/csrc/kp1_tracker.inc b/rl_brain_trainer_amd/csrc/kp1_tracker.inc
--- /dev/null
+++ b/rl_brain_trainer_amd/csrc/kp1_tracker.inc
@@ -0,0 +1,313 @@
+struct TrackerCtx {
+  int stage, count, len, head, window, min_episodes, max_stage, n_events, sum;
+  double threshold;
+  long long timesteps;
+  bool ring_dirty;
+};
+
+__device__ __forceinline__ void trk_wave_sync() {
+  __builtin_amdgcn_fence(__ATOMIC_RELEASE, "workgroup");
+  __builtin_amdgcn_wave_barrier();
+  __builtin_amdgcn_fence(__ATOMIC_ACQUIRE, "workgroup");
+}
+
+struct TrackerEvents { kp1_curriculum_event* a; kp1_curriculum_event* b; };
+__device__ __forceinline__ void tracker_record(const TrackerEvents& evs, int n_events, long long timesteps, int stage, double rate) {
+  if (n_events >= KP1_CURRICULUM_MAX_HISTORY) return;
+  kp1_curriculum_event* const dst[2] = {evs.a, evs.b};
+#pragma unroll
+  for (int k = 0; k < 2; ++k)
+    if (dst[k]) {
+      kp1_curriculum_event& ev = dst[k][n_events];
+      ev.total_timesteps = timesteps;
+      ev.from_stage = stage;
+      ev.to_stage = stage + 1;
+      ev.trigger_success_rate = rate;
+    }
+}
+
+__device__ __forceinline__ void tracker_load(const kp1_curriculum_state* st, int* __restrict__ ring, TrackerCtx& c, const int lane) {
+  c.stage = st->stage_index; c.count = st->stage_episode_count; c.len = st->ring_len; c.head = st->ring_head;
+  c.window = st->window_episodes; c.min_episodes = st->min_episodes_per_stage; c.max_stage = st->max_stage_index; c.n_events = st->n_events;
+  c.threshold = st->success_rate_threshold; c.timesteps = st->num_timesteps;
+  c.ring_dirty = false;
+  int part = 0;
+  for (int k = lane; k < c.window; k += 64) {
+    const int v = st->ring[k];
+    ring[k] = v;
+    const int age = k >= c.head ? k - c.head : k - c.head + c.window;
+    if (age < c.len) part += v;
+  }
+  for (int off = 32; off > 0; off >>= 1) part += __shfl_xor(part, off);
+  c.sum = part;
+  trk_wave_sync();
+}
+
+__device__ __forceinline__ void tracker_store(kp1_curriculum_state* st, const int* __restrict__ ring, const TrackerCtx& c, const int lane, const bool whole) {
+  trk_wave_sync();
+  if (c.ring_dirty || whole)
+    for (int k = lane; k < c.window; k += 64) st->ring[k] = ring[k];
+  if (lane == 0) {
+    st->stage_index = c.stage; st->stage_episode_count = c.count; st->ring_len = c.len; st->ring_head = c.head;
+    st->n_events = c.n_events; st->num_timesteps = c.timesteps;
+    if (whole) {
+      st->window_episodes = c.window; st->min_episodes_per_stage = c.min_episodes; st->max_stage_index = c.max_stage;
+      st->success_rate_threshold = c.threshold;
+    }
+  }
+}
+
+constexpr int TRK_BLOCK = 64 * 64, TRK_PARALLEL_MIN = 192;
+struct TrackerScratch { uint8_t* sbit; uint16_t* pfx; };
+constexpr int TRK_LDS_RING = KP1_CURRICULUM_MAX_WINDOW * 4, TRK_LDS_SBIT = TRK_BLOCK;
+constexpr int TRK_LDS_PFX = ((TRK_BLOCK + KP1_CURRICULUM_MAX_WINDOW + 1) * 2 + 15) / 16 * 16;
+constexpr int TRK_LDS_BYTES = TRK_LDS_RING + TRK_LDS_SBIT + TRK_LDS_PFX;
+
+__device__ __forceinline__ void tracker_append_run(int* __restrict__ ring, TrackerCtx& c, const uint8_t* __restrict__ sbit, int pos, int R, const int lane) {
+  const int W = c.window;
+  const int j0 = R > W ? R - W : 0;
+  trk_wave_sync();
+  for (int j = j0 + lane; j < R; j += 64) ring[(c.head + c.len + j) % W] = sbit[pos + j];
+  trk_wave_sync();
+  const int over = c.len + R - W;
+  c.head = over > 0 ? (c.head + over) % W : c.head;
+  c.len = c.len + R < W ? c.len + R : W;
+  c.count += R;
+  int part = 0;
+  for (int k = lane; k < W; k += 64) {
+    const int age = k >= c.head ? k - c.head : k - c.head + W;
+    if (age < c.len) part += ring[k];
+  }
+  for (int off = 32; off > 0; off >>= 1) part += __shfl_xor(part, off);
+  c.sum = part;
+}
+
+__device__ __forceinline__ void tracker_block_parallel(const TrackerEvents& evs, int* __restrict__ ring, TrackerCtx& c, const TrackerScratch& ws,
+                                                       unsigned long long dmask, unsigned long long smask, int E, const int lane) {
+  const int W = c.window;
+  int mine = __popcll(dmask), off = mine;
+  for (int d = 1; d < 64; d <<= 1) {
+    const int up = __shfl_up(off, d);
+    if (lane >= d) off += up;
+  }
+  off -= mine;
+  trk_wave_sync();
+  for (unsigned long long m = dmask; m; m &= m - 1) {
+    const int b = __ffsll((long long)m) - 1;
+    ws.sbit[off++] = (uint8_t)((smask >> b) & 1ull);
+  }
+  trk_wave_sync();
+  int pos = 0;
+  while (pos < E) {
+    const int R = E - pos;
+    if (c.stage >= c.max_stage) {
+      tracker_append_run(ring, c, ws.sbit, pos, R, lane);
+      break;
+    }
+    const int L = c.len, T = L + R;
+    const int seg = (T + 63) / 64, j_lo = lane * seg < T ? lane * seg : T, j_hi = j_lo + seg < T ? j_lo + seg : T;
+    auto y = [&](int j) -> int { return j < L ? ring[(c.head + j) % W] : (int)ws.sbit[pos + (j - L)]; };
+    int tot = 0;
+    for (int j = j_lo; j < j_hi; ++j) tot += y(j);
+    int run = tot;
+    for (int d = 1; d < 64; d <<= 1) {
+      const int up = __shfl_up(run, d);
+      if (lane >= d) run += up;
+    }
+    run -= tot;
+    trk_wave_sync();
+    if (lane == 0) ws.pfx[0] = 0;
+    for (int j = j_lo; j < j_hi; ++j) {
+      run += y(j);
+      ws.pfx[j + 1] = (uint16_t)run;
+    }
+    trk_wave_sync();
+    int best = R;
+    for (int r = lane; r < R; r += 64) {
+      const int filled = L + r + 1;
+      if (filled < W || c.count + r + 1 < c.min_episodes) continue;
+      const int wsum = (int)ws.pfx[filled] - (int)ws.pfx[filled - W];
+      if ((double)wsum / (double)W >= c.threshold) {
+        best = r;
+        break;
+      }
+    }
+    for (int d = 32; d > 0; d >>= 1) {
+      const int o = __shfl_xor(best, d);
+      best = o < best ? o : best;
+    }
+    if (best >= R) {
+      tracker_append_run(ring, c, ws.sbit, pos, R, lane);
+      break;
+    }
+    const int filled = L + best + 1;
+    const double rate = (double)((int)ws.pfx[filled] - (int)ws.pfx[filled - W]) / (double)W;
+    if (lane == 0) tracker_record(evs, c.n_events, c.timesteps, c.stage, rate);
+    c.n_events += 1;
+    c.stage += 1;
+    c.count = 0;
+    c.len = 0;
+    c.head = 0;
+    c.sum = 0;
+    pos += best + 1;
+  }
+}
+
+__device__ __forceinline__ void curriculum_scan(const TrackerEvents& evs, int* __restrict__ ring, TrackerCtx& c, const TrackerScratch& ws,
+                                                const uint8_t* __restrict__ dones, int n, int steps_per_call, const int lane) {
+  c.timesteps += steps_per_call;
+  for (int base = 0; base < n; base += 64 * 64) {
+    const int first = base + lane * 64;
+    unsigned long long dmask = 0ull, smask = 0ull;
+    if (first + 64 <= n && (reinterpret_cast<uintptr_t>(dones + first) & 15) == 0) {
+      const uint4* p = reinterpret_cast<const uint4*>(dones + first);
+      uint4 w[4];
+#pragma unroll
+      for (int q = 0; q < 4; ++q) w[q] = p[q];
+#pragma unroll
+      for (int q = 0; q < 4; ++q) {
+        const unsigned int words[4] = {w[q].x, w[q].y, w[q].z, w[q].w};
+#pragma unroll
+        for (int k = 0; k < 4; ++k)
+#pragma unroll
+          for (int b = 0; b < 4; ++b) {
+            const unsigned int d = (words[k] >> (8 * b)) & 0xffu;
+            const int bit = q * 16 + k * 4 + b;
+            if (d & (KP1_DONE_TERMINATED | KP1_DONE_TRUNCATED)) {
+              dmask |= 1ull << bit;
+              if (d & KP1_DONE_SUCCESS) smask |= 1ull << bit;
+            }
+          }
+      }
+    } else {
+      for (int b = 0; b < 64 && first + b < n; ++b) {
+        const uint8_t d = dones[first + b];
+        if (d & (KP1_DONE_TERMINATED | KP1_DONE_TRUNCATED)) {
+          dmask |= 1ull << b;
+          if (d & KP1_DONE_SUCCESS) smask |= 1ull << b;
+        }
+      }
+    }
+    unsigned long long busy = __ballot(dmask != 0ull);
+    if (busy == 0ull) continue;
+    c.ring_dirty = true;
+    {
+      int ended = __popcll(dmask);
+      for (int off = 32; off > 0; off >>= 1) ended += __shfl_xor(ended, off);
+      if (ended >= TRK_PARALLEL_MIN) {
+        tracker_block_parallel(evs, ring, c, ws, dmask, smask, ended, lane);
+        continue;
+      }
+    }
+    int stage = c.stage, count = c.count, len = c.len, head = c.head, sum = c.sum, n_events = c.n_events;
+    const int window = c.window;
+    trk_wave_sync();
+    while (busy) {
+      const int src = __ffsll((long long)busy) - 1;
+      busy &= busy - 1;
+      unsigned long long m = __shfl(dmask, src);
+      const unsigned long long sm = __shfl(smask, src);
+      if (lane != 0) continue;
+      while (m) {
+        const int b = __ffsll((long long)m) - 1;
+        m &= m - 1;
+        const int success = (int)((sm >> b) & 1ull);
+        count += 1;
+        if (len < window) {
+          ring[head + len < window ? head + len : head + len - window] = success;
+          len += 1;
+          sum += success;
+        } else {
+          sum += success - ring[head];
+          ring[head] = success;
+          head = head + 1 < window ? head + 1 : 0;
+        }
+        if (stage >= c.max_stage) continue;
+        if (count < c.min_episodes) continue;
+        if (len < window) continue;
+        const double rate = (double)sum / (double)len;
+        if (rate >= c.threshold) {
+          tracker_record(evs, n_events, c.timesteps, stage, rate);
+          n_events += 1;
+          stage += 1;
+          count = 0;
+          len = 0;
+          head = 0;
+          sum = 0;
+        }
+      }
+    }
+    c.stage = __shfl(stage, 0); c.count = __shfl(count, 0); c.len = __shfl(len, 0); c.head = __shfl(head, 0);
+    c.sum = __shfl(sum, 0); c.n_events = __shfl(n_events, 0);
+  }
+}
+
+struct TrackerAhead { uint4 w[4]; bool wide; };
+__device__ __forceinline__ TrackerAhead tracker_fetch(const uint8_t* __restrict__ dones, int n, const int lane) {
+  TrackerAhead h;
+  const int first = lane * 64;
+  h.wide = first + 64 <= n && (reinterpret_cast<uintptr_t>(dones + first) & 15) == 0;
+#pragma unroll
+  for (int q = 0; q < 4; ++q) h.w[q] = h.wide ? reinterpret_cast<const uint4*>(dones + first)[q] : uint4{0u, 0u, 0u, 0u};
+  return h;
+}
+__device__ __forceinline__ bool tracker_any_done(const TrackerAhead& h, const uint8_t* __restrict__ dones, int n, const int lane) {
+  bool any = false;
+  for (int base = 0; base < n; base += 64 * 64) {
+    const int first = base + lane * 64;
+    if (base == 0 && h.wide) {
+      unsigned int acc = 0u;
+#pragma unroll
+      for (int q = 0; q < 4; ++q) acc |= h.w[q].x | h.w[q].y | h.w[q].z | h.w[q].w;
+      any |= (acc & (0x01010101u * (unsigned)(KP1_DONE_TERMINATED | KP1_DONE_TRUNCATED))) != 0u;
+    } else if (first + 64 <= n && (reinterpret_cast<uintptr_t>(dones + first) & 15) == 0) {
+      const uint4* p = reinterpret_cast<const uint4*>(dones + first);
+      unsigned int acc = 0u;
+#pragma unroll
+      for (int q = 0; q < 4; ++q) {
+        const uint4 w = p[q];
+        acc |= w.x | w.y | w.z | w.w;
+      }
+      any |= (acc & (0x01010101u * (unsigned)(KP1_DONE_TERMINATED | KP1_DONE_TRUNCATED))) != 0u;
+    } else {
+      for (int b = 0; b < 64 && first + b < n; ++b) any |= (dones[first + b] & (KP1_DONE_TERMINATED | KP1_DONE_TRUNCATED)) != 0;
+    }
+  }
+  return __ballot(any) != 0ull;
+}
+
+template <typename Publish>
+__device__ __forceinline__ void tracker_observe_wave(const kp1_curriculum_state* st_in, kp1_curriculum_state* st_out, const bool store,
+                                                     const TrackerAhead& ahead, const uint8_t* __restrict__ dones, int n, int steps_per_call,
+                                                     const int lane, char* lds, Publish publish) {
+  const bool whole = st_out != st_in;
+  const int stage_in = st_in->stage_index;
+  if (!tracker_any_done(ahead, dones, n, lane)) {
+    publish(stage_in);
+    if (store && !whole) {
+      if (lane == 0) atomicAdd(reinterpret_cast<unsigned long long*>(&st_out->num_timesteps), (unsigned long long)(long long)steps_per_call);
+      return;
+    }
+    if (store) {
+      const int window = st_in->window_episodes;
+      for (int k = lane; k < window; k += 64) st_out->ring[k] = st_in->ring[k];
+      if (lane == 0) {
+        st_out->stage_index = st_in->stage_index; st_out->stage_episode_count = st_in->stage_episode_count;
+        st_out->ring_len = st_in->ring_len; st_out->ring_head = st_in->ring_head;
+        st_out->window_episodes = window; st_out->min_episodes_per_stage = st_in->min_episodes_per_stage;
+        st_out->max_stage_index = st_in->max_stage_index; st_out->n_events = st_in->n_events;
+        st_out->success_rate_threshold = st_in->success_rate_threshold;
+        st_out->num_timesteps = st_in->num_timesteps + steps_per_call;
+      }
+    }
+    return;
+  }
+  int* ring = reinterpret_cast<int*>(lds);
+  const TrackerScratch ws = {reinterpret_cast<uint8_t*>(lds + TRK_LDS_RING), reinterpret_cast<uint16_t*>(lds + TRK_LDS_RING + TRK_LDS_SBIT)};
+  const TrackerEvents evs = {store ? st_out->events : nullptr, store && whole ? const_cast<kp1_curriculum_state*>(st_in)->events : nullptr};
+  TrackerCtx c;
+  tracker_load(st_in, ring, c, lane);
+  curriculum_scan(evs, ring, c, ws, dones, n, steps_per_call, lane);
+  publish(c.stage);
+  if (store) tracker_store(st_out, ring, c, lane, whole);
+}
diff --git a/rl_brain_trainer_amd/curriculum.py b/rl_brain_trainer_amd/curriculum.py
--- a/rl_brain_trainer_amd/curriculum.py
+++ b/rl_brain_trainer_amd/curriculum.py
@@ -24,6 +24,10 @@
     ]
 
 
+class TrackerFold(C.Structure):
+    _fields_ = [("state_in", C.c_void_p), ("state_out", C.c_void_p), ("prev_dones", C.c_void_p), ("steps_per_call", C.c_int32)]
+
+
 class PointCurriculum:
     def __init__(self, *, success_rate_threshold: float, window_episodes: int, min_episodes_per_stage: int, max_stage_index: int,
                  initial_stage_index: int = 0, device: torch.device | int = 0) -> None:
@@ -44,6 +48,22 @@
         stream = torch.cuda.current_stream(self.device).cuda_stream
         native.check(self.L.kp1_curriculum_observe(self.device.index or 0, self._st, C.c_void_p(dones.data_ptr()), int(dones.numel()),
                                                    int(steps_per_call), C.c_void_p(stream)))
+
+    def _pair(self, k: int) -> int:
+        if k & 1 == 0:
+            return int(self._st.value)
+        if getattr(self, "_second", None) is None:
+            self._second = torch.zeros(C.sizeof(CurriculumState), dtype=torch.uint8, device=self.device)
+        return self._second.data_ptr()
+
+    def fold(self, t: int, prev_dones: torch.Tensor, steps_per_call: int) -> TrackerFold:
+        assert t >= 1 and prev_dones.dtype == torch.uint8 and prev_dones.is_contiguous()
+        return TrackerFold(self._pair(t - 1), self._pair(t), prev_dones.data_ptr(), int(steps_per_call))
+
+    def fold_close(self, n_steps: int, dones: torch.Tensor, steps_per_call: int) -> None:
+        stream = torch.cuda.current_stream(self.device).cuda_stream
+        native.check(self.L.kp1_curriculum_observe_from(self.device.index or 0, C.c_void_p(self._pair(n_steps - 1)), self._st, C.c_void_p(dones.data_ptr()),
+                                                        int(dones.numel()), int(steps_per_call), C.c_void_p(stream)))
 
     def observe_chunk(self, dones_all: torch.Tensor, n_local: int, chunk_steps: int, world: int) -> None:
         assert dones_all.numel() == world * chunk_steps * n_local and dones_all.dtype == torch.uint8 and dones_all.is_contiguous()
diff --git a/rl_brain_trainer_amd/mlp.py b/rl_brain_trainer_amd/mlp.py
--- a/rl_brain_trainer_amd/mlp.py
+++ b/rl_brain_trainer_amd/mlp.py
@@ -27,7 +27,7 @@
         L.kp1_mlp_num_params_ex.restype = C.c_int64
         L.kp1_mlp_pack_weights.argtypes = [vp, vp, vp]
         L.kp1_mlp_forward.argtypes = [vp, vp, i32, i32, vp, vp, vp, vp, vp, vp, vp]
-        L.kp1_mlp_forward_env_step.argtypes = [vp, vp, vp, i32, vp, vp, vp, vp, vp, vp, vp, vp, vp]
+        L.kp1_mlp_forward_env_step.argtypes = [vp, vp, vp, i32, vp, vp, vp, vp, vp, vp, vp, vp, vp, vp]
         L.kp1_mlp_loss_grad.argtypes = [vp, vp, i32, vp, i32, vp, vp, vp, vp, f32, f32, vp, f32, f32, f32, f32, vp, vp, i32, vp]
         L.kp1_mlp_adam_step.argtypes = [vp, vp, vp, vp, vp, f32, f32, f32, i32, i32, vp]
         L.kp1_mlp_time_kernels.argtypes = [vp, vp, i32, i32, i32, vp, vp, vp]
@@ -107,10 +107,11 @@
         assert obs.is_contiguous() and obs.dtype == torch.float32
         native.check(self.L.kp1_mlp_forward(self._h, _p(obs), stride, n, _p(noise), _p(mean), _p(value), _p(action), _p(clipped), _p(log_prob), self._stream()))
 
-    def forward_env_step(self, env, obs: torch.Tensor, *, noise, value, action, log_prob, next_obs, reward, done, terminal_obs) -> None:
+    def forward_env_step(self, env, obs: torch.Tensor, *, noise, value, action, log_prob, next_obs, reward, done, terminal_obs, tracker=None) -> None:
         assert obs.is_contiguous() and obs.dtype == torch.float32 and obs.shape[0] == env.n_envs
         native.check(self.L.kp1_mlp_forward_env_step(self._h, env._handle, _p(obs), obs.shape[1], _p(noise), _p(value), _p(action), _p(log_prob),
-                                                     _p(next_obs), _p(reward), _p(done), _p(terminal_obs), self._stream()))
+                                                     _p(next_obs), _p(reward), _p(done), _p(terminal_obs), self._stream(),
+                                                     C.cast(C.pointer(tracker), C.c_void_p) if tracker is not None else None))
 
     def mean_value(self, obs: torch.Tensor) -> tuple[torch.Tensor, torch.Tensor]:
         n = obs.shape[0]
diff --git a/rl_brain_trainer_amd/native.py b/rl_brain_trainer_amd/native.py
--- a/rl_brain_trainer_amd/native.py
+++ b/rl_brain_trainer_amd/native.py
@@ -94,6 +94,7 @@
     L.kp1_curriculum_create.argtypes = [i32, C.c_double, i32, i32, i32, i32, C.POINTER(vp)]
     L.kp1_curriculum_destroy.argtypes = [i32, vp]
     L.kp1_curriculum_observe.argtypes = [i32, vp, vp, i32, i32, vp]
+    L.kp1_curriculum_observe_from.argtypes = [i32, vp, vp, vp, i32, i32, vp]
     L.kp1_curriculum_observe_chunk.argtypes = [i32, vp, vp, i32, i32, i32, vp]
     L.kp1_curriculum_read.argtypes = [i32, vp, vp, vp]
     L.kp1_bind_stage_ptr.argtypes = [vp, vp]
diff --git a/rl_brain_trainer_amd/ppo.py b/rl_brain_trainer_amd/ppo.py
--- a/rl_brain_trainer_amd/ppo.py
+++ b/rl_brain_trainer_amd/ppo.py
@@ -413,6 +413,11 @@
         self._fused_env_step = bool(type(env) is ArmKinematicVecEnv and env.dtype == torch.float32 and cfg.hidden == 256
                                     and self.obs_dim <= 64 and not getattr(env, "_reward_components_on", False)
                                     and os.environ.get("KP1_FUSED_ROLLOUT", "1") != "0")
+        self._tracker_fold = bool(self._fused_env_step and not self.dist.enabled and type(curriculum) is PointCurriculum
+                                  and self.n_envs <= self.TRACKER_FOLD_MAX_ENVS and os.environ.get("KP1_TRACKER_FOLD", "1") != "0")
+
+    TRACKER_FOLD_MAX_ENVS = 8192
+    _tracker_fold = False
 
     def _setup(self, cfg: PPOConfig, seeds: list[int], envs: list[Any], curricula: list[Any], dist: Dist, use_graphs: bool, *,
                min_batch: int, stacked: bool) -> None:
@@ -633,14 +638,20 @@
                                          C.c_void_p(self.adv_buf.data_ptr()), C.c_void_p(self.ret_buf.data_ptr()), T, KN, C.c_void_p(stream)))
 
     def _rollout_step_hip(self, t: int) -> None:
+        if self._tracker_fold and self.env._mode_name == "approach":
+            cur = self.curriculum
+            self._policy_env_step(t, cur.fold(t, self.done_buf[t - 1], self.n_envs) if t > 0 else None)
+            if t == self.cfg.n_steps - 1:
+                cur.fold_close(self.cfg.n_steps, self.done_buf[t], self.n_envs)
+            return
         self._policy_env_step(t)
         self._curriculum_observe(t)
 
-    def _policy_env_step(self, t: int) -> None:
+    def _policy_env_step(self, t: int, tracker=None) -> None:
         if self._fused_env_step:
             self._mlp.forward_env_step(self.env, self.obs_buf[t], noise=self.noise_all[t], value=self.val_buf[t], action=self.act_buf[t],
                                        log_prob=self.logp_buf[t], next_obs=self.obs_buf[t + 1], reward=self.rew_buf[t], done=self.done_buf[t],
-                                       terminal_obs=self.term_obs_buf[t])
+                                       terminal_obs=self.term_obs_buf[t], tracker=tracker)
         else:
             self._mlp.forward(self.obs_buf[t], noise=self.noise_all[t], value=self.val_buf[t], action=self.act_buf[t],
                               clipped=self.clip_act, log_prob=self.logp_buf[t])
```

After: 11.43 million (median of 4 runs). No clear change (+0.3%).
